# chlhnu/DOT-SOCP

Hardware: AMD Instinct MI355X
Metric: ADMM iters/sec on NxNxT dot2d staggered grid at 1/2/4/8 MI355X (higher is better)
Workload: dtype f64

## Files before the change

dot-socp_amd/capi.py:

```python
import ctypes
import os

import numpy as np

_HERE = os.path.dirname(os.path.abspath(__file__))
LIB_PATH = os.path.join(_HERE, "lib", "libdotsocp.so")

i64 = ctypes.c_longlong
dbl = ctypes.c_double
vp = ctypes.c_void_p


class DotsocpError(RuntimeError):
    def __init__(self, code, msg):
        super().__init__(f"libdotsocp error {code}: {msg}")
        self.code = code


class Problem(ctypes.Structure):
    _fields_ = [("dim", ctypes.c_int), ("weighted", ctypes.c_int),
                ("ny", i64), ("nx", i64), ("nt", i64),
                ("D", dbl), ("E", dbl), ("cScale", dbl), ("dScale", dbl),
                ("normc", dbl), ("normd", dbl)]


class Opts(ctypes.Structure):
    _fields_ = [("tau", dbl), ("sigma", dbl), ("tol", dbl), ("maxit", i64),
                ("ifCheckStepByStep", ctypes.c_int), ("checkPrimDualFeas", ctypes.c_int),
                ("scaling", ctypes.c_int), ("time_limit", dbl)]


class Result(ctypes.Structure):
    _fields_ = [("sigma", dbl), ("sigma_internal", dbl), ("cScale", dbl), ("dScale", dbl),
                ("times", dbl * 7), ("iters", i64), ("hist_len", i64), ("stopped", ctypes.c_int),
                ("time_extra", dbl)]


class AccOpts(ctypes.Structure):
    _fields_ = [("restart", i64), ("rho", dbl), ("theta", dbl)]


METHOD_INPALM, METHOD_PALM, METHOD_ACCADMM = 0, 1, 2


F_PHI, F_Q, F_ALPHA, F_Z, F_BETA, F_C, F_WEIGHT = range(7)

SYMBOLS = {
    "dotsocp_last_error": (ctypes.c_char_p, []),
    "dotsocp_version": (ctypes.c_char_p, []),
    "dotsocp_device_count": (ctypes.c_int, []),
    "dotsocp_proj_soc": (ctypes.c_int, [vp, vp, i64, i64]),
    "dotsocp_bfd": (ctypes.c_int, [vp, vp, i64, i64, i64, dbl, dbl]),
    "dotsocp_bfd_conj": (ctypes.c_int, [vp, vp, i64, i64, i64, dbl]),
    "dotsocp_bfd1d": (ctypes.c_int, [vp, vp, i64, i64, dbl, dbl]),
    "dotsocp_bfd_conj1d": (ctypes.c_int, [vp, vp, i64, i64, dbl]),
    "dotsocp_oper_poisson": (ctypes.c_int, [vp, vp, i64, i64, i64, dbl]),
    "dotsocp_dctn": (ctypes.c_int, [vp, i64, i64, i64, ctypes.c_int]),
    "dotsocp_proj_soc_dev": (ctypes.c_int, [vp, vp, i64, i64, vp]),
    "dotsocp_bfd_dev": (ctypes.c_int, [vp, vp, i64, i64, i64, dbl, dbl, vp]),
    "dotsocp_bfd_conj_dev": (ctypes.c_int, [vp, vp, i64, i64, i64, dbl, vp]),
    "dotsocp_create": (vp, [ctypes.POINTER(Problem), ctypes.c_int, ctypes.c_int]),
    "dotsocp_create_multi": (vp, [ctypes.POINTER(Problem), ctypes.c_int, ctypes.c_int]),
    "dotsocp_destroy": (None, [vp]),
    "dotsocp_rccl_unique_id": (ctypes.c_int, [vp]),
    "dotsocp_attach_rccl": (ctypes.c_int, [vp, vp, ctypes.c_int, ctypes.c_int]),
    "dotsocp_slab_range": (ctypes.c_int, [i64, ctypes.c_int, ctypes.c_int, ctypes.POINTER(i64), ctypes.POINTER(i64)]),
    "dotsocp_field_len": (i64, [ctypes.POINTER(Problem), ctypes.c_int]),
    "dotsocp_dct_algorithm": (ctypes.c_int, [i64]),
    "dotsocp_release_cache": (i64, []),
    "dotsocp_upload": (ctypes.c_int, [vp, ctypes.c_int, vp]),
    "dotsocp_upload_layers": (ctypes.c_int, [vp, ctypes.c_int, vp, i64, i64]),
    "dotsocp_download": (ctypes.c_int, [vp, ctypes.c_int, vp]),
    "dotsocp_begin": (ctypes.c_int, [vp, ctypes.POINTER(Opts)]),
    "dotsocp_begin_method": (ctypes.c_int, [vp, ctypes.POINTER(Opts), ctypes.c_int, ctypes.POINTER(AccOpts)]),
    "dotsocp_run": (ctypes.c_int, [vp, i64, ctypes.POINTER(i64)]),
    "dotsocp_recover_outputs": (ctypes.c_int, [vp, vp, vp, vp, vp, vp, vp, vp, vp]),
    "dotsocp_jump_next_level": (ctypes.c_int, [vp, vp]),
    "dotsocp_finish": (ctypes.c_int, [vp, ctypes.POINTER(Result)]),
    "dotsocp_get_history": (ctypes.c_int, [vp, vp, vp, vp, vp]),
    "dotsocp_set_profiling": (ctypes.c_int, [vp, ctypes.c_int]),
    "dotsocp_kernel_time": (ctypes.c_int, [vp, ctypes.c_char_p, ctypes.POINTER(dbl), ctypes.POINTER(i64)]),
    "dotsocp_canary_check": (ctypes.c_int, []),
    "dotsocp_synchronize": (ctypes.c_int, [vp]),
}

_lib = None


def _share_torchs_hip_runtime():
    import importlib.util
    import sys
    if "torch" in sys.modules or os.environ.get("DOTSOCP_SYSTEM_HIP"):
        return
    try:
        spec = importlib.util.find_spec("torch")
    except (ImportError, ValueError):
        return
    if not spec or not spec.submodule_search_locations:
        return
    for name in ("libamdhip64.so", "libamdhip64.so.7"):
        path = os.path.join(list(spec.submodule_search_locations)[0], "lib", name)
        if os.path.exists(path):
            try:
                ctypes.CDLL(path, mode=ctypes.RTLD_GLOBAL)
            except OSError:
                pass
            return


def lib():
    global _lib
    if _lib is None:
        _share_torchs_hip_runtime()
        if not os.path.exists(LIB_PATH):
            raise ImportError(
                f"{LIB_PATH} is missing: build the HIP extension first "
                "(python -c 'import __graft_entry__ as g; g.build()'); there is no CPU fallback")
        L = ctypes.CDLL(LIB_PATH)
        for name, (res, args) in SYMBOLS.items():
            f = getattr(L, name)
            f.restype = res
            f.argtypes = args
        _lib = L
    return _lib


def check(code):
    if code != 0:
        raise DotsocpError(code, lib().dotsocp_last_error().decode())


def fptr(a):
    if not isinstance(a, np.ndarray) or a.dtype != np.float64 or not (a.flags.f_contiguous or a.flags.c_contiguous):
        raise ValueError("expected a contiguous float64 numpy array")
    return a.ctypes.data


def slab_range(nt, world, rank):
    t0, t1 = i64(), i64()
    check(lib().dotsocp_slab_range(nt, world, rank, ctypes.byref(t0), ctypes.byref(t1)))
    return t0.value, t1.value


def rccl_unique_id():
    buf = (ctypes.c_ubyte * 128)()
    check(lib().dotsocp_rccl_unique_id(buf))
    return bytes(buf)


DCT_ALGORITHMS = ("none", "fft", "pfa", "rader", "bluestein", "dense")

# ... 4 lines not shown
```

dot-socp_amd/csrc/capi.hip:

```cpp
#include <cstring>
#include <new>

#include "comm.h"
#include "solver.h"

using namespace dotsocp;

namespace dotsocp {
extern thread_local std::string g_last_error;
int dotsocp_slab_range_impl(i64 nt, int world, int rank, i64 *t0, i64 *t1);
}

struct dotsocp_ctx {
    Solver s;
};

static int require_device() {
    int n = 0;
    if (hipGetDeviceCount(&n) != hipSuccess || n <= 0) {
        set_error("no HIP device available (libdotsocp has no CPU fallback)");
        return DOTSOCP_ENODEVICE;
    }
    return 0;
}
// ... 171 lines not shown
    DS_ARG(res && rhs && ny >= 1 && nx >= 1 && nt >= 1, "bad array");
    DS_CHECK(require_device());
    const i64 n = ny * nx * nt;
    DevBuf da, db, cy, cx, ct;
    Plans pl;
    DS_CHECK(da.alloc(n));
    DS_CHECK(db.alloc(n));
    DS_CHECK(pl.make(ny, nx, nt));
    const double pi = 3.14159265358979323846;
    auto table = [&](DevBuf &d, i64 m) -> int {
        std::vector<double> t((size_t)m);
        for (i64 k = 0; k < m; ++k) t[k] = (2.0 * (double)(m - 1) * (double)(m - 1)) * (1.0 - cos(pi * (double)k / (double)m));
        DS_CHECK(d.alloc(m));
        DS_HIP(hipMemcpy(d.p, t.data(), sizeof(double) * m, hipMemcpyHostToDevice));
        return 0;
    };
    DS_CHECK(table(cy, ny));
    DS_CHECK(table(cx, nx));
    DS_CHECK(table(ct, nt));
    DS_HIP(hipMemcpy(da.p, rhs, sizeof(double) * n, hipMemcpyHostToDevice));
    Grid g;
    g.set(ny, nx, nt, 0, nt);
    DS_CHECK(launch_dct_axis(pl.py, da.p, db.p, ny, nx, nt, 0, 0, nullptr));
    DS_CHECK(launch_dct_axis(pl.px, db.p, da.p, ny, nx, nt, 1, 0, nullptr));
    DS_CHECK(launch_poisson_t_single(pl.pt, g, kernelScale, cy.p, cx.p, ct.p, da.p, db.p, 0, nullptr, tsolve_tri_allowed()));
    DS_CHECK(launch_dct_axis(pl.px, da.p, db.p, ny, nx, nt, 1, 1, nullptr));
    DS_CHECK(launch_dct_axis(pl.py, db.p, da.p, ny, nx, nt, 0, 1, nullptr));
    DS_HIP(hipDeviceSynchronize());
    DS_HIP(hipMemcpy(res, da.p, sizeof(double) * n, hipMemcpyDeviceToHost));
    return 0;
}

dotsocp_ctx *dotsocp_create(const dotsocp_problem *prob, int device, int nslabs) {
    dotsocp_ctx *c = new (std::nothrow) dotsocp_ctx();
    if (!c) { set_error("out of host memory"); return nullptr; }
    if (c->s.init(prob, device, nslabs) != 0) {
        delete c;
        return nullptr;
    }
    return c;
}

dotsocp_ctx *dotsocp_create_multi(const dotsocp_problem *prob, int first_device, int ngpu) {
    dotsocp_ctx *c = new (std::nothrow) dotsocp_ctx();
    if (!c) { set_error("out of host memory"); return nullptr; }
    if (c->s.init(prob, first_device, ngpu, true) != 0) {
        delete c;
        return nullptr;
    }
    return c;
}

void dotsocp_destroy(dotsocp_ctx *ctx) { delete ctx; }

int dotsocp_slab_range(dotsocp_i64 nt, int world, int rank, dotsocp_i64 *t0, dotsocp_i64 *t1) {
    DS_ARG(t0 && t1 && world >= 1 && rank >= 0 && rank < world && nt >= 2 * world, "bad slab request");
    return dotsocp_slab_range_impl(nt, world, rank, t0, t1);
}

int dotsocp_rccl_unique_id(unsigned char id[128]) {
    DS_ARG(id != nullptr, "id is NULL");
    Rccl &api = rccl_api();
    DS_CHECK(api.load());
    ncclUniqueId uid;
    static_assert(sizeof(uid) == 128, "ncclUniqueId is expected to be 128 bytes");
    DS_NCCL(api.GetUniqueId(&uid));
    memcpy(id, &uid, sizeof uid);
    return 0;
}

int dotsocp_attach_rccl(dotsocp_ctx *ctx, const unsigned char id[128], int rank, int world) {
    if (!ctx) { set_error("ctx is NULL"); return DOTSOCP_EINVAL; }
    return ctx->s.attach_rccl(id, rank, world);
}

#define CTX_OR_FAIL()                                      \
    do {                                                   \
        if (!ctx) { set_error("ctx is NULL"); return DOTSOCP_EINVAL; } \
        (void)hipGetLastError();    \
    } while (0)

int dotsocp_dct_algorithm(dotsocp_i64 n) { return dct_choose_algorithm(n); }

dotsocp_i64 dotsocp_field_len(const dotsocp_problem *p, int field) {
    if (!p || (p->dim != 1 && p->dim != 2) || p->nt < 2 || p->nx < 1 || (p->dim == 2 && p->ny < 1)) return -1;
    const i64 ny = p->dim == 1 ? p->nx : p->ny, nx = p->dim == 1 ? 1 : p->nx, nt = p->nt;
    const i64 Nphi = ny * nx * nt, Nz = ny * nx * (nt - 1);
    const i64 Nq = Nz + ny * (nx - 1) * nt + (ny - 1) * nx * nt;
    switch (field) {
        case DOTSOCP_F_PHI: case DOTSOCP_F_C: return Nphi;
        case DOTSOCP_F_Q: case DOTSOCP_F_ALPHA: case DOTSOCP_F_WEIGHT: return Nq;
        case DOTSOCP_F_Z: case DOTSOCP_F_BETA: return Nz * (p->dim == 1 ? 6 : 10);
        default: return -1;
    }
}

int dotsocp_upload(dotsocp_ctx *ctx, int field, const double *host) { CTX_OR_FAIL(); return ctx->s.upload(field, host); }
dotsocp_i64 dotsocp_release_cache(void) { return (dotsocp_i64)device_cache_release(); }

int dotsocp_upload_layers(dotsocp_ctx *ctx, int field, const double *host, dotsocp_i64 t0, dotsocp_i64 n) {
    CTX_OR_FAIL();
    return ctx->s.upload_layers(field, host, t0, n);
}
int dotsocp_download(dotsocp_ctx *ctx, int field, double *host) { CTX_OR_FAIL(); return ctx->s.download(field, host); }
int dotsocp_begin(dotsocp_ctx *ctx, const dotsocp_opts *opts) { CTX_OR_FAIL(); return ctx->s.begin(opts); }
int dotsocp_begin_method(dotsocp_ctx *ctx, const dotsocp_opts *opts, int method, const dotsocp_acc_opts *acc) {
    CTX_OR_FAIL();
    return ctx->s.begin_method(opts, method, acc);
}
int dotsocp_recover_outputs(dotsocp_ctx *ctx, const double *rho0, const double *rho1, double *rho, double *Ex,
                            double *Ey, double *q0, double *bx, double *by) {
    CTX_OR_FAIL();
    if (ctx->s.prob.dim == 1)
        return ctx->s.recover_outputs(rho0, rho1, rho, nullptr, Ex, q0, nullptr, bx);
    return ctx->s.recover_outputs(rho0, rho1, rho, Ex, Ey, q0, bx, by);
}

int dotsocp_jump_next_level(dotsocp_ctx *coarse, dotsocp_ctx *fine) {
    if (!coarse || !fine) { set_error("context is NULL"); return DOTSOCP_EINVAL; }
    return fine->s.jump_from(coarse->s);
}

int dotsocp_run(dotsocp_ctx *ctx, dotsocp_i64 n_iters, dotsocp_i64 *done) { CTX_OR_FAIL(); return ctx->s.run(n_iters, done); }
int dotsocp_finish(dotsocp_ctx *ctx, dotsocp_result *res) { CTX_OR_FAIL(); return ctx->s.finish(res); }

int dotsocp_get_history(dotsocp_ctx *ctx, double *kkt, double *time, double *iter, double *pdGap) {
    CTX_OR_FAIL();
    const Solver &s = ctx->s;
    const size_t n = s.hist_iter.size();
    for (size_t i = 0; i < n; ++i) {
        if (kkt) for (int j = 0; j < 7; ++j) kkt[j * n + i] = s.hist_kkt[i * 7 + j];
        if (time) time[i] = s.hist_time[i];
        if (iter) iter[i] = s.hist_iter[i];
        if (pdGap) pdGap[i] = s.hist_gap[i];
    }
    return 0;
}

int dotsocp_set_profiling(dotsocp_ctx *ctx, int on) {
    CTX_OR_FAIL();
    ctx->s.profiling = on != 0;
    return 0;
}

int dotsocp_kernel_time(dotsocp_ctx *ctx, const char *name, double *avg_ms, dotsocp_i64 *launches) {
    CTX_OR_FAIL();
    DS_ARG(name != nullptr, "name is NULL");
    static const char *names[PH_COUNT] = {"rhs", "poisson", "cone_proj", "qstep", "beta", "kkt",
                                          "cone_fused_a", "cone_fused_b", "materialise", "comm",
                                          "interp", "acc_cone", "acc_gather", "qstep_first", "transpose"};
    for (int i = 0; i < PH_COUNT; ++i)
        if (strcmp(name, names[i]) == 0) {
            const i64 n = ctx->s.phase_launches[i];
            if (avg_ms) *avg_ms = n ? ctx->s.phase_ms[i] / (double)n : 0.0;
            if (launches) *launches = n;
            return 0;
        }
    set_error("unknown kernel family '%s'", name);
    return DOTSOCP_EINVAL;
}

int dotsocp_canary_check(void) {
    std::string rep;
    const int bad = canary_check(&rep);
    if (bad) set_error("canary: %d device buffer(s) written out of bounds: %s", bad, rep.c_str());
    return bad;
}

int dotsocp_synchronize(dotsocp_ctx *ctx) {
    CTX_OR_FAIL();
    ctx->s.cur_dev = -1;
    return ctx->s.sync_all();
}

}
```

dot-socp_amd/csrc/cone.hip:

```cpp
#include "device_utils.h"
#include "kernels.h"

namespace dotsocp {


template <int K>
__global__ void __launch_bounds__(256) k_proj_soc(double *__restrict__ out, const double *__restrict__ in, i64 M) {
    for (i64 i = (i64)blockIdx.x * blockDim.x + threadIdx.x; i < M; i += (i64)gridDim.x * blockDim.x) {
        double v[K];
#pragma unroll
        for (int j = 0; j < K; ++j) v[j] = in[j * M + i];
        proj_row<K>(v);
#pragma unroll
        for (int j = 0; j < K; ++j) out[j * M + i] = v[j];
    }
}

__global__ void __launch_bounds__(256) k_proj_soc_any(double *__restrict__ out, const double *__restrict__ in, i64 M,
                                                      i64 K) {
    for (i64 i = (i64)blockIdx.x * blockDim.x + threadIdx.x; i < M; i += (i64)gridDim.x * blockDim.x) {
        double x1 = in[i];
        const double n = sqrt(soc_norm2([&](i64 j) { return in[j * M + i]; }, K));
        double c = (x1 / n + 1.0) * 0.5;
        c = (c > 1.0) ? 1.0 : c;
// ... 30 lines not shown
    const double q0 = q[i];
    z[i] = dF - s * q0;
    z[9 * g.Nc + i] = dF + s * q0;
    const double *bx = q + g.offBx;
    const double *by = q + g.offBy;
#pragma unroll
    for (int dt = 0; dt < 2; ++dt) {
        const i64 tt = tl + dt;
        if (x >= 1) z[(1 + 2 * dt) * g.Nc + i] = sf * bx[g.bxLayer * tt + y + g.py * (x - 1)];
        if (x <= g.nx - 2) z[(2 + 2 * dt) * g.Nc + i] = sf * bx[g.bxLayer * tt + y + g.py * x];
        if (y >= 1) z[(5 + 2 * dt) * g.Nc + i] = sf * by[g.byLayer * tt + (y - 1) + g.pyb * x];
        if (y <= g.ny - 2) z[(6 + 2 * dt) * g.Nc + i] = sf * by[g.byLayer * tt + y + g.pyb * x];
    }
}

int launch_bfd(const Grid &g, double *z, const double *q, double s, double dF, hipStream_t st) {
    if (g.Nz <= 0) return 0;
    DS_KLAUNCH(k_bfd, cell_grid(g, g.ncl), dim3(TILE_Y, TILE_X), 0, st, g, z, q, s, edge_factor(s), dF);
    DS_HIP(hipGetLastError());
    return 0;
}

__global__ void __launch_bounds__(TILE_Y *TILE_X) k_bfd_conj(Grid g, double *__restrict__ q, const double *__restrict__ w,
                                                              double s, double sf, int seg,
                                                              const double *__restrict__ tail_bx,
                                                              const double *__restrict__ tail_by) {
    const i64 y = (i64)blockIdx.x * TILE_Y + threadIdx.x;
    const i64 x = (i64)blockIdx.y * TILE_X + threadIdx.y;
    const i64 tl = blockIdx.z;
    WPlain W{w, g.Nc};
    if (seg == 0) {
        if (y >= g.ny || x >= g.nx) return;
        const i64 i = y + g.py * (x + g.nx * tl);
        q[i] = s * (w[9 * g.Nc + i] - w[i]);
    } else if (seg == 1) {
        if (y >= g.ny || x >= g.nx - 1) return;
        q[g.offBx + g.bxLayer * tl + y + g.py * x] = sf * gather_bx(g, W, y, x, tl, tail_bx);
    } else {
        if (y >= g.ny - 1 || x >= g.nx) return;
        q[g.offBy + g.byLayer * tl + y + g.pyb * x] = sf * gather_by(g, W, y, x, tl, tail_by);
    }
}

int launch_bfd_conj(const Grid &g, double *q, const double *w, double s, hipStream_t st, const double *tail_bx,
                    const double *tail_by) {
    const double sf = edge_factor(s);
    if (!g.first && (!tail_bx || !tail_by)) {
        set_error("bfd_conj on a time slab needs the left neighbour's tails");
        return DOTSOCP_EINVAL;
    }
    const dim3 blk(TILE_Y, TILE_X);
    if (g.Nz > 0) DS_KLAUNCH(k_bfd_conj, cell_grid(g, g.ncl), blk, 0, st, g, q, w, s, sf, 0, tail_bx, tail_by);
    if (g.bxLayer > 0) DS_KLAUNCH(k_bfd_conj, cell_grid(g, g.ntl), blk, 0, st, g, q, w, s, sf, 1, tail_bx, tail_by);
    if (g.byLayer > 0) DS_KLAUNCH(k_bfd_conj, cell_grid(g, g.ntl), blk, 0, st, g, q, w, s, sf, 2, tail_bx, tail_by);
    DS_HIP(hipGetLastError());
    return 0;
}

#define MARCH 8

template <int MODE>
__global__ void __launch_bounds__(TILE_Y *TILE_X) k_cone_march(Grid g, LoopCoef c, const double *__restrict__ q,
                                                                const double *zin, const double *betain,
                                                                double *zout, double *betaout) {
    const i64 y = (i64)blockIdx.x * TILE_Y + threadIdx.x;
    const i64 x = (i64)blockIdx.y * TILE_X + threadIdx.y;
    if (y >= g.ny || x >= g.nx) return;
    const i64 tbeg = (i64)blockIdx.z * MARCH;
    const i64 tend = (tbeg + MARCH < g.ncl) ? tbeg + MARCH : g.ncl;
    EdgeQuad cur = load_edges(g, q, y, x, tbeg, c.sf);
    for (i64 tl = tbeg; tl < tend; ++tl) {
        const i64 i = y + g.py * (x + g.nx * tl);
        const EdgeQuad nxt = load_edges(g, q, y, x, tl + 1, c.sf);
        double v[10];
        build_z2(v, q[i], cur, nxt, c.s, c.dF);
        if (MODE == 0) {
#pragma unroll
            for (int j = 0; j < 10; ++j) v[j] = v[j] - betain[j * g.Nc + i];
            proj_row<10>(v);
#pragma unroll
            for (int j = 0; j < 10; ++j) zout[j * g.Nc + i] = v[j];
        } else {
#pragma unroll
            for (int j = 0; j < 10; ++j) {
                const double r = zin[j * g.Nc + i] - v[j];
                betaout[j * g.Nc + i] = betain[j * g.Nc + i] + c.tau * r;
            }
        }
        cur = nxt;
    }
}

static inline dim3 march_grid(const Grid &g) {
    return dim3((unsigned)((g.ny + TILE_Y - 1) / TILE_Y), (unsigned)((g.nx + TILE_X - 1) / TILE_X),
                (unsigned)((g.ncl + MARCH - 1) / MARCH));
}

int launch_cone_proj(const Grid &g, const LoopCoef &c, const double *q, const double *beta, double *z,
                     hipStream_t st) {
    if (g.Nz <= 0) return 0;
    DS_KLAUNCH(k_cone_march<0>, march_grid(g), dim3(TILE_Y, TILE_X), 0, st, g, c, q, (const double *)nullptr,
                       beta, z, (double *)nullptr);
    DS_HIP(hipGetLastError());
    return 0;
}

int launch_beta_update(const Grid &g, const LoopCoef &c, const double *q, const double *z, double *beta,
                       hipStream_t st) {
    if (g.Nz <= 0) return 0;
    DS_KLAUNCH(k_cone_march<1>, march_grid(g), dim3(TILE_Y, TILE_X), 0, st, g, c, q, z, (const double *)beta,
                       (double *)nullptr, beta);
    DS_HIP(hipGetLastError());
    return 0;
}

__global__ void __launch_bounds__(TILE_Y *TILE_X) k_gather_tail(Grid g, const double *__restrict__ z,
                                                                 const double *__restrict__ beta,
                                                                 double *__restrict__ tail_bx,
                                                                 double *__restrict__ tail_by) {
    const i64 y = (i64)blockIdx.x * TILE_Y + threadIdx.x;
    const i64 x = (i64)blockIdx.y * TILE_X + threadIdx.y;
    const i64 tl = g.ncl - 1;
    auto w = [&](int j, i64 cell) { return z[j * g.Nc + cell] + beta[j * g.Nc + cell]; };
    if (y < g.ny && x < g.nx - 1) {
        double acc = w(3, y + g.py * ((x + 1) + g.nx * tl));
        acc += w(4, y + g.py * (x + g.nx * tl));
        tail_bx[y + g.py * x] = acc;
    }
    if (y < g.ny - 1 && x < g.nx) {
        double acc = w(7, (y + 1) + g.py * (x + g.nx * tl));
        acc += w(8, y + g.py * (x + g.nx * tl));
        tail_by[y + g.pyb * x] = acc;
    }
}

int launch_gather_tail(const Grid &g, const double *z, const double *beta, double *tail_bx, double *tail_by,
                       hipStream_t st) {
    if (g.ncl <= 0) return 0;
    DS_KLAUNCH(k_gather_tail, cell_grid(g, 1), dim3(TILE_Y, TILE_X), 0, st, g, z, beta, tail_bx, tail_by);
    DS_HIP(hipGetLastError());
    return 0;
}

}
```

dot-socp_amd/csrc/device_utils.h:

```cpp
#pragma once
#include "common.h"

namespace dotsocp {

#define TILE_Y 64
#define TILE_X 4

__device__ __forceinline__ i64 xcd_tile(unsigned b, unsigned nb) {
    const unsigned full = nb >> 3, rem = nb & 7u, r = b & 7u, q = b >> 3;
    return (i64)r * full + (r < rem ? r : rem) + q;
}

struct BlockId {
    unsigned x, y, z;
};
__device__ __forceinline__ BlockId block_id(bool remap) {
    BlockId b{blockIdx.x, blockIdx.y, blockIdx.z};
    if (remap) {
        const unsigned nb = gridDim.x * gridDim.y * gridDim.z;
        const i64 L = xcd_tile(b.x + gridDim.x * (b.y + gridDim.y * b.z), nb);
        b.x = (unsigned)(L % gridDim.x);
        b.y = (unsigned)((L / gridDim.x) % gridDim.y);
        b.z = (unsigned)(L / ((i64)gridDim.x * gridDim.y));
    }
    return b;
}

__device__ __forceinline__ void lds_barrier() { asm volatile("s_waitcnt lgkmcnt(0)\n\ts_barrier" ::: "memory"); }

__device__ __forceinline__ void glds16(const void *gsrc, unsigned lds_dst) {
    unsigned keep;
    asm volatile("s_mov_b32 %0, m0\n\ts_mov_b32 m0, %2\n\ts_nop 0\n\tglobal_load_lds_dwordx4 %1, off\n\ts_mov_b32 m0, %0"
                 : "=&s"(keep)
                 : "v"(gsrc), "s"(lds_dst)
                 : "memory");
}

template <bool NT>
__device__ __forceinline__ double ld_stream(const double *p) { return NT ? __builtin_nontemporal_load(p) : *p; }
template <bool NT>
__device__ __forceinline__ void st_stream(double *p, double v) {
    if (NT) __builtin_nontemporal_store(v, p);
    else *p = v;
}
bool stream_nt_enabled();

template <class X, class I>
__device__ __forceinline__ double soc_norm2(const X &x, I K) {
    const I lim = (K - 2) & ~(I)3;
    double p = x(1) * x(1);
    I j = 2;
#pragma unroll
    for (; j - 1 < lim; j += 4) {
        const double a = x(j), b = x(j + 1), c = x(j + 2), d = x(j + 3);
        p += (a * a + b * b) + (c * c + d * d);
    }
#pragma unroll
    for (; j < K; ++j) p += x(j) * x(j);
    return p;
}

template <int K>
__device__ __forceinline__ void proj_row(double (&v)[K]) {
    const double n = sqrt(soc_norm2([&](int j) { return v[j]; }, K));
    double c = (v[0] / n + 1.0) * 0.5;
    c = (c > 1.0) ? 1.0 : c;
    c = (c < 0.0) ? 0.0 : c;
#pragma unroll
    for (int j = 1; j < K; ++j) v[j] = c * v[j];
    v[0] = (c >= 1.0) ? v[0] : c * n;
}

struct EdgeQuad {
    double xm, xp, ym, yp;
};

__device__ __forceinline__ EdgeQuad load_edges(const Grid &g, const double *__restrict__ q, i64 y, i64 x,
                                               i64 tt, double sf) {
    const double *bx = (g.nx >= 2) ? q + g.offBx + g.bxLayer * tt : q;
    const double *by = (g.ny >= 2) ? q + g.offBy + g.byLayer * tt : q;
    const i64 nxe = (g.nx >= 2) ? g.nx - 2 : 0, nye = (g.ny >= 2) ? g.ny - 2 : 0;
    const i64 rowy = (g.ny >= 2) ? g.pyb : 0;
    const i64 xm = (x >= 1) ? x - 1 : 0, xp = (x <= nxe) ? x : nxe;
    const i64 ym = (y >= 1) ? y - 1 : 0, yp = (y <= nye) ? y : nye;
    const double vxm = bx[y + g.py * xm], vxp = bx[y + g.py * xp];
    const double vym = by[ym + rowy * x], vyp = by[yp + rowy * x];
    EdgeQuad e;
    e.xm = (x >= 1) ? sf * vxm : 0.0;
    e.xp = (x <= g.nx - 2) ? sf * vxp : 0.0;
    e.ym = (y >= 1) ? sf * vym : 0.0;
    e.yp = (y <= g.ny - 2) ? sf * vyp : 0.0;
    return e;
}

__device__ __forceinline__ void build_z2(double (&v)[10], double q0, const EdgeQuad &a, const EdgeQuad &b,
                                         double s, double dF) {
    v[0] = dF - s * q0;
    v[1] = a.xm; v[2] = a.xp; v[3] = b.xm; v[4] = b.xp;
    v[5] = a.ym; v[6] = a.yp; v[7] = b.ym; v[8] = b.yp;
    v[9] = dF + s * q0;
}

template <class W>
__device__ __forceinline__ double gather_bx(const Grid &g, const W &w, i64 y, i64 xe, i64 tl,
                                            const double *__restrict__ tail_bx) {
    double acc = 0.0;
    if (tl < g.ncl) {
        acc += w(1, y + g.py * ((xe + 1) + g.nx * tl));
        acc += w(2, y + g.py * (xe + g.nx * tl));
    }
    if (tl >= 1) {
        acc += w(3, y + g.py * ((xe + 1) + g.nx * (tl - 1)));
        acc += w(4, y + g.py * (xe + g.nx * (tl - 1)));
    } else if (!g.first) {
        acc += tail_bx[y + g.py * xe];
    }
    return acc;
}

template <class W>
__device__ __forceinline__ double gather_by(const Grid &g, const W &w, i64 ye, i64 x, i64 tl,
                                            const double *__restrict__ tail_by) {
    double acc = 0.0;
    if (tl < g.ncl) {
        acc += w(5, (ye + 1) + g.py * (x + g.nx * tl));
        acc += w(6, ye + g.py * (x + g.nx * tl));
    }
    if (tl >= 1) {
        acc += w(7, (ye + 1) + g.py * (x + g.nx * (tl - 1)));
        acc += w(8, ye + g.py * (x + g.nx * (tl - 1)));
    } else if (!g.first) {
        acc += tail_by[ye + g.pyb * x];
    }
    return acc;
}

struct WPlain {
    const double *w;
    i64 Nz;
    __device__ __forceinline__ double operator()(int j, i64 cell) const { return w[j * Nz + cell]; }
};

struct RhsArgs {
    Grid g;
    double at, ax, ay;
    const double *q, *alpha, *cvec, *weight, *u0_prev;
};

template <bool WEIGHTED>
__device__ __forceinline__ double rhs_value(const RhsArgs &a, i64 y, i64 x, i64 tl) {
    const Grid &g = a.g;
    auto u = [&](i64 k) { return WEIGHTED ? a.weight[k] * a.q[k] - a.alpha[k] : a.q[k] - a.alpha[k]; };
    const i64 node = y + g.py * (x + g.nx * tl);
    double r = 0.0;
    if (tl >= 1)
        r += a.at * u(node - g.plane);
    else if (!g.first)
        r += a.at * a.u0_prev[y + g.py * x];
    if (tl < g.ncl) r += (-a.at) * u(node);
    const i64 bxo = g.offBx + g.bxLayer * tl;
    if (x >= 1) r += a.ax * u(bxo + y + g.py * (x - 1));
    if (x <= g.nx - 2) r += (-a.ax) * u(bxo + y + g.py * x);
    const i64 byo = g.offBy + g.byLayer * tl;
    if (y >= 1) r += a.ay * u(byo + (y - 1) + g.pyb * x);
    if (y <= g.ny - 2) r += (-a.ay) * u(byo + y + g.pyb * x);
    return r + a.cvec[node];
}

}
```

dot-socp_amd/csrc/fused.hip:

```cpp
#include "device_utils.h"
#include "gather_tile.h"
#include "kernels.h"

#include <cstdlib>

namespace dotsocp {

template <int MODE, int XB, bool NT = false>
__global__ void __launch_bounds__(64 * XB) k_cone_fused(Grid g, LoopCoef c, FusedArgs a) {
    constexpr bool DUAL = (MODE >= 5);
    constexpr bool UPD = (MODE != 0 && MODE != 6);
    constexpr bool PROJ = (MODE < 2 || MODE >= 5);
    __shared__ double2 xch[2][XB][64];
    __shared__ double2 xchp[DUAL ? 2 : 1][DUAL ? XB : 1][DUAL ? 64 : 1];
    const int lane = threadIdx.x, xl = threadIdx.y;
    const BlockId blk = block_id(a.xcd != 0);
    const i64 y = (i64)blk.x * 64 + lane;
    const i64 x = (i64)blk.y * XB + xl;
    const bool inb = (y < g.ny) && (x < g.nx);
    const i64 yc = inb ? y : 0, xc = inb ? x : 0;
    const i64 t0 = ((i64)blk.z + a.z0) * a.TC;
    const i64 t1 = (t0 + a.TC < g.ncl) ? t0 + a.TC : g.ncl;
    const bool lastChunk = (t1 == g.ncl);
    constexpr bool GATHER = (PROJ || MODE == 4);
    const bool carried = GATHER && !DUAL && t0 > 0 && a.carry_in != nullptr;
    const i64 tstart = (GATHER && t0 > 0 && !carried) ? t0 - 1 : t0;
    const i64 nxblk = gridDim.y, nyblk = gridDim.x;

    EdgeQuad cur = load_edges(g, a.q, yc, xc, tstart, c.sf), curo, cur3;
    if (UPD) curo = load_edges(g, a.q_old, yc, xc, tstart, c.sf);
    if (MODE == 5) cur3 = load_edges(g, a.q3, yc, xc, tstart, c.sf);
    GatherCarry gc, gcp;
    if (carried) {
        const i64 ci = yc + g.py * xc;
        gc.p3 = a.carry_in[ci]; gc.p4 = a.carry_in[g.plane + ci];
        gc.p7 = a.carry_in[2 * g.plane + ci]; gc.p8 = a.carry_in[3 * g.plane + ci];
    }
    const i64 tstop = (GATHER && lastChunk) ? t1 + 1 : t1;
    for (i64 tl = tstart; tl < tstop; ++tl) {
        const bool hasCell = tl < g.ncl;
        const bool own = tl >= t0;
        double w[10], wp[10];
        if (hasCell) {
            const i64 i = yc + g.py * (xc + g.nx * tl);
            const EdgeQuad nxt = load_edges(g, a.q, yc, xc, tl + 1, c.sf);
            double b[10], v[10];
#pragma unroll
            for (int j = 0; j < 10; ++j) b[j] = ld_stream<NT>(a.beta_in + j * g.Nc + i);
            if (a.bpend) {
#pragma unroll
                for (int j = 0; j < 10; ++j) b[j] = b[j] * a.bmul / a.bdiv;
                if (a.bpend > 1) {
#pragma unroll
                    for (int j = 0; j < 10; ++j) b[j] = b[j] * a.bmul2 / a.bdiv2;
                }
            }
            build_z2(v, a.q[i], cur, nxt, c.s, c.dF);
            if (UPD) {
                const EdgeQuad nxto = load_edges(g, a.q_old, yc, xc, tl + 1, c.sf);
                double zo[10];
                build_z2(zo, a.q_old[i], curo, nxto, c.s, c.dF);
#pragma unroll
                for (int j = 0; j < 10; ++j) zo[j] = zo[j] - b[j];
                proj_row<10>(zo);
#pragma unroll
                for (int j = 0; j < 10; ++j) {
                    const double r = zo[j] - v[j];
                    b[j] = b[j] + c.tau * r;
                }
                if (own && inb) {
                    if (MODE != 3) {
#pragma unroll
                        for (int j = 0; j < 10; ++j) st_stream<NT>(a.beta_out + j * g.Nc + i, b[j]);
                    }
                    if (MODE == 2 || MODE == 3) {
#pragma unroll
                        for (int j = 0; j < 10; ++j) st_stream<NT>(a.z_out + j * g.Nc + i, zo[j]);
                    }
                }
                curo = nxto;
                if (MODE == 4) {
#pragma unroll
                    for (int j = 0; j < 10; ++j) w[j] = zo[j] + b[j];
                    if (own && inb) a.q2[i] = c.s * (w[9] - w[0]);
                }
            }
            cur = nxt;
            if (PROJ) {
                if (MODE == 5) {
                    const EdgeQuad nxt3 = load_edges(g, a.q3, yc, xc, tl + 1, c.sf);
                    build_z2(v, a.q3[i], cur3, nxt3, c.s, c.dF);
                    cur3 = nxt3;
                }
#pragma unroll
                for (int j = 0; j < 10; ++j) v[j] = v[j] - b[j];
                proj_row<10>(v);
#pragma unroll
                for (int j = 0; j < 10; ++j) w[j] = v[j] + b[j];
                if (own && inb) a.q2[i] = c.s * (w[9] - w[0]);
                if (DUAL) {
#pragma unroll
                    for (int j = 0; j < 10; ++j) wp[j] = w[j] + c.tau * v[j];
                    if (own && inb) a.p2[i] = c.s * (wp[9] - wp[0]);
                }
            }
        } else {
#pragma unroll
            for (int j = 0; j < 10; ++j) w[j] = 0.0;
            if (DUAL) {
#pragma unroll
                for (int j = 0; j < 10; ++j) wp[j] = 0.0;
            }
        }
        if constexpr (GATHER && !DUAL)
            gather_emit<XB>(g, c.sf, xch, gc, w, tl, own && inb, x, y, xl, lane, nxblk, nyblk, blk.y, blk.x,
                            a.q2, a.sx, a.sy);
        if constexpr (DUAL) {
            gather_post<XB>(xch, gc, w, xl, lane);
            gather_post<XB>(xchp, gcp, wp, xl, lane);
            __syncthreads();
            gather_finish<XB>(g, c.sf, xch, gc, w, tl, own && inb, x, y, xl, lane, nxblk, nyblk, blk.y, blk.x,
                              a.q2, a.sx, a.sy);
            gather_finish<XB>(g, c.sf, xchp, gcp, wp, tl, own && inb, x, y, xl, lane, nxblk, nyblk, blk.y, blk.x,
                              a.p2, a.sxp, a.syp);
        }
    }
    if (GATHER && !DUAL && !lastChunk && a.carry_out != nullptr && inb) {
        const i64 ci = y + g.py * x;
        a.carry_out[ci] = gc.p3; a.carry_out[g.plane + ci] = gc.p4;
        a.carry_out[2 * g.plane + ci] = gc.p7; a.carry_out[3 * g.plane + ci] = gc.p8;
    }
}

bool stream_nt_enabled() {
    const char *e = getenv("DOTSOCP_NT");
    return !(e && atoi(e) == 0);
}

bool tile_xcd_remap(const Grid &g) {
    return (g.py % 16) != 0;
}

bool cone_split_enabled() { return true; }

int fused_geometry(const Grid &g, FusedGeom &fg) {
    fg.XB = 4;
    fg.nyblk = (g.ny + 63) / 64;
    fg.nxblk = (g.nx + fg.XB - 1) / fg.XB;
    const i64 tiles = fg.nyblk * fg.nxblk;
    const i64 target = 2048;
    i64 chunks = (target + tiles - 1) / tiles;
    if (chunks < 1) chunks = 1;
    if (!(g.first && g.last) && cone_split_enabled() && chunks < 2 && g.ncl >= 12) chunks = 2;
    i64 TC = (g.ncl + chunks - 1) / chunks;
    if (TC < 8) TC = 8;
    if (TC > g.ncl) TC = g.ncl;
    if (TC < 1) TC = 1;
    fg.TC = TC;
    fg.chunks = (g.ncl + TC - 1) / TC;
    fg.sx_len = (g.ncl + 1) * fg.nxblk * g.ny;
    fg.sy_len = (g.ncl + 1) * g.nx * fg.nyblk;
    return 0;
}

int launch_cone_fused(int mode, const Grid &g, const LoopCoef &c, const FusedGeom &fg, FusedArgs a,
                      hipStream_t st, i64 z0, i64 zcount) {
    if (g.Nz <= 0) return 0;
    if (zcount < 0) zcount = fg.chunks - z0;
    if (z0 < 0 || zcount <= 0 || z0 + zcount > fg.chunks) return 0;
    a.TC = fg.TC;
    a.z0 = (int)z0;
    a.xcd = tile_xcd_remap(g) ? 1 : 0;
    dim3 grid((unsigned)fg.nyblk, (unsigned)fg.nxblk, (unsigned)zcount);
    dim3 blk(64, 4);
    const bool nt = stream_nt_enabled();
#define CONE_MODE(M)                                                                     \
    case M:                                                                              \
        if (nt) DS_KLAUNCH((k_cone_fused<M, 4, true>), grid, blk, 0, st, g, c, a);       \
        else DS_KLAUNCH((k_cone_fused<M, 4>), grid, blk, 0, st, g, c, a);                \
        break;
    switch (mode) {
        CONE_MODE(0) CONE_MODE(1) CONE_MODE(2) CONE_MODE(3) CONE_MODE(4) CONE_MODE(5) CONE_MODE(6)
#undef CONE_MODE
        default: set_error("bad fused mode"); return DOTSOCP_EINVAL;
    }
    DS_HIP(hipGetLastError());
    return 0;
}

}
```

dot-socp_amd/csrc/kernels.h:

```cpp
#pragma once
#include "common.h"
#include "defer.h"

namespace dotsocp {

struct LoopCoef {
    double s;
    double sf;
    double dF;
    double at, ax, ay;
    double tau;
    double c1, c2;
    double dinv1, dinv2;
};

enum {
    S_Q2 = 0, S_Z2, S_APHI2, S_ALPHA2, S_BETA2, S_FBBETA2, S_PRIM1, S_PRIM2, S_DUAL1, S_DUAL2,
    S_COMPLEM, S_DOTCOMP, S_RHO2, S_RHOFQ2, S_MRHOB, S_M2, S_RHOB2, S_QALPHA, S_CPHI, S_PHI2,
    S_COUNT
};

struct KktCoef {
    double sigma;
    double kappa;
    double dsD;
    double dsE;
};

int launch_proj_soc(double *out, const double *in, i64 M, i64 K, hipStream_t st);
int launch_bfd(const Grid &g, double *z, const double *q, double s, double dF, hipStream_t st);
int launch_bfd_conj(const Grid &g, double *q, const double *w, double s, hipStream_t st, const double *tail_bx = nullptr,
                    const double *tail_by = nullptr);
int launch_cone_proj(const Grid &g, const LoopCoef &c, const double *q, const double *beta, double *z,
                     hipStream_t st);
int launch_beta_update(const Grid &g, const LoopCoef &c, const double *q, const double *z, double *beta,
                       hipStream_t st);
int launch_gather_tail(const Grid &g, const double *z, const double *beta, double *tail_bx, double *tail_by,
                       hipStream_t st);

struct FusedGeom {
    int XB;
    i64 nyblk, nxblk;
    i64 TC, chunks;
    i64 sx_len, sy_len;
};
struct FusedArgs {
    const double *q_old;
    const double *q;
    const double *beta_in;
    double *beta_out;
    double *z_out;
    double *q2;
    double *sx, *sy;
    const double *q3;
    double *p2, *sxp, *syp;
    i64 TC;
    int bpend;
    double bmul, bdiv;
    double bmul2, bdiv2;
    int xcd;
    int z0;
    const double *carry_in;
    double *carry_out;
};
bool tile_xcd_remap(const Grid &g);
int fused_geometry(const Grid &g, FusedGeom &fg);
int launch_cone_fused(int mode, const Grid &g, const LoopCoef &c, const FusedGeom &fg, FusedArgs a,
                      hipStream_t st, i64 z0 = 0, i64 zcount = -1);
bool cone_split_enabled();

struct KktWork;
struct AccArgs {
    const double *q;
    const double *z_in, *beta_in;
    const double *z0, *beta0;
    double *z0_out, *beta0_out;
    double bdiv;
    KktCoef kk;
    const double *alpha_p, *weight;
    double *partials;
    int nostore;
    double *z_out, *beta_out;
    double *q2, *sx, *sy;
    i64 TC;
    double c1, c2, om_rho, rho;
};
struct AccCoef {
    double c1, c2, om_rho, rho;
    double om_c1, c1c2;
};
int launch_acc_cone(int mode, const Grid &g, const LoopCoef &c, const FusedGeom &fg, AccArgs a, hipStream_t st);
int launch_acc_cone_kkt(const Grid &g, const LoopCoef &c, const FusedGeom &fg, AccArgs a, const KktWork &w, hipStream_t st);
int launch_acc_restart(double *x, const double *xp, double *anchor, i64 n, const AccCoef &k, double div, hipStream_t st);
int launch_acc_interp(double *x, const double *xp, double *aux, i64 n, const AccCoef &k, int mode, int write_aux,
                      hipStream_t st);

int launch_prolong_phi(const Grid &gf, const Grid &gc, const double *phic, double *phif, double sc_in, double sc_out,
                       hipStream_t st, i64 tc0 = 0);
int launch_prolong_beta(const Grid &gf, const Grid &gc, const double *betac, double *betaf, double *neg, double sc_in0,
                        double sc_in1, double sc_out, hipStream_t st, i64 tc0 = 0, i64 Nzc = -1);
int launch_scale_div(double *x, const double *w, i64 n, double sc, hipStream_t st);
int launch_fill(double *x, i64 n, double v, hipStream_t st);
int launch_outputs(const Grid &g, const double *q, const double *alpha, const double *weight, const double *rho0,
                   const double *rho1, const double *a_prev, double sig, double cD, double dD, int which, double *out,
                   hipStream_t st);
int launch_out_tail(const Grid &g, const double *alpha, const double *weight, double sig, double cD, double *out,
                    hipStream_t st);

int launch_qstep_fused(const Grid &g, const LoopCoef &c, const FusedGeom &fg, const double *phi,
                       const double *q2, const double *sx, const double *sy, const double *weight,
                       const double *tail_bx, const double *tail_by, double *q_out, double *alpha,
                       hipStream_t st);
struct QStepExtra {
    int apend;
    double amul, adiv;
    double *partials, *resid;
    double kappa, dsD;
    double *u0_tail;
};
int launch_qstep_rhs(const Grid &g, const LoopCoef &c, const FusedGeom &fg, const double *phi, const double *q2,
                     const double *sx, const double *sy, const double *weight, const double *tail_bx,
                     const double *tail_by, const double *cvec, double *q_out, const double *alpha_in, double *alpha_out,
                     double *rhs, hipStream_t st, i64 z0 = 0, i64 zcount = -1, i64 zstride = 1,
                     const QStepExtra *ex = nullptr);
i64 qstep_rhs_blocks(const Grid &g, const FusedGeom &fg);
int launch_rhs_sigma_fix(double *rhs, const double *r, double *cvec, i64 n, double factor, hipStream_t st);
i64 qstep_rhs_chunks(const Grid &g, const FusedGeom &fg, i64 *TC = nullptr);
int launch_qstep_rhs_acc(int var, const Grid &g, const LoopCoef &c, const FusedGeom &fg, const double *phi,
                         const double *q2, const double *sx, const double *sy, const double *weight, const double *cvec,
                         double *q_raw, const double *alpha_in, double *alpha_out, double *rhs, double *q_state,
                         const double *q_anchor, const double *alpha_anchor, const AccCoef &k, hipStream_t st,
                         const double *tail_bx = nullptr, const double *tail_by = nullptr, double *u0_tail = nullptr);
int launch_rhs_fixup(const Grid &g, const LoopCoef &c, const double *u0_prev, double *rhs, hipStream_t st);
int launch_qstep_palm_first(const Grid &g, const LoopCoef &c, const FusedGeom &fg, const double *phi, const double *q2,
                            const double *sx, const double *sy, const double *cvec, double *q_out, const double *alpha,
                            double *rhs, hipStream_t st, const double *tail_bx = nullptr, const double *tail_by = nullptr,
                            const double *qk = nullptr);
int launch_grad(const Grid &g, const LoopCoef &c, const double *phi, double *out, hipStream_t st);
int launch_tail_finalize(const Grid &g, const LoopCoef &c, const FusedGeom &fg, const double *q2, const double *sx,
                         const double *sy, double *tail_bx, double *tail_by, hipStream_t st);
int launch_kkt_tail(const Grid &g, const double *alpha, const double *beta, const double *weight, double *a0,
                    double *a0w, double *bt_bx, double *bt_by, hipStream_t st);
int launch_rhs(const Grid &g, const LoopCoef &c, const double *q, const double *alpha, const double *cvec,
               const double *weight, const double *u0_prev, double *rhs, hipStream_t st);
int launch_qstep(const Grid &g, const LoopCoef &c, const double *phi, const double *z, const double *beta,
                 const double *weight, const double *tail_bx, const double *tail_by, double *q,
                 double *alpha, hipStream_t st);
int launch_u0_tail(const Grid &g, const double *q, const double *alpha, const double *weight, double *out,
                   hipStream_t st);
int launch_scale(double *x, i64 n, double mul, double div, hipStream_t st);
#define DS_MAX_WORLD 64
struct PencilCuts {
    int world;
    i64 cut[DS_MAX_WORLD + 1];
};
int launch_pencil_pack(bool pack, const PencilCuts &pc, i64 plane, i64 ntl, double *slab, double *stage, hipStream_t st);

#define TRI_EXTRA 256
int launch_tri_local(const Grid &g, i64 nt, double kscale, const double *cy, const double *cx, const PencilCuts &pc,
                     const double *r, double *send, hipStream_t st);
int launch_tri_reduced(const Grid &g, i64 nt, double kscale, const double *cy, const double *cx, const PencilCuts &pc,
                       int rank, i64 l0, i64 nl, const i64 *slab_n, const double *recv, double *back, double *zero_work,
                       hipStream_t st, const double *own_recv = nullptr, double *own_back = nullptr);
int launch_tri_final(const Grid &g, i64 nt, double kscale, const double *cy, const double *cx, const PencilCuts &pc,
                     const double *back, double *x, hipStream_t st);
bool tsolve_tri_supported(i64 nt);
bool tsolve_tri_preferred(i64 nt, bool pow2, i64 plane);
int launch_tsolve_tri(const Grid &g, i64 nt, double kscale, const double *cy, const double *cx, double *x, hipStream_t st);
struct GatherMsgs {
    const double *src[DS_MAX_WORLD];
    double *dst[DS_MAX_WORLD];
    i64 count[DS_MAX_WORLD];
    int n;
};
int launch_gather_msgs(const GatherMsgs &m, hipStream_t st);

#define KKT_SLICES 64
struct KktWork {
    double *partials;
    i64 maxBlocks;
    double *sums;
};
struct KktHalo {
    const double *a0_prev, *a0w_prev, *btail_bx, *btail_by;
};
i64 kkt_partials_needed(const Grid &g);
int launch_kkt(const Grid &g, const LoopCoef &c, const KktCoef &k, const double *phi, const double *q,
               const double *alpha, const double *z, const double *beta, const double *cvec,
               const double *weight, const KktHalo &halo, const KktWork &w, int parts, hipStream_t st,
               bool layer0 = false, double *resid = nullptr);
int launch_kkt_nodual(const Grid &g, const LoopCoef &c, const KktCoef &k, const double *phi, const double *q,
                      const double *alpha, const double *cvec, const double *weight, const KktWork &w, hipStream_t st);
int launch_kkt_bnd_dual(const Grid &g, const LoopCoef &c, const KktCoef &k, const FusedGeom &fg, const double *q,
                        const double *alpha, const double *weight, const double *q2, const double *sx, const double *sy,
                        const KktWork &w, hipStream_t st);
int launch_kkt_cells_update(const Grid &g, const LoopCoef &c, const KktCoef &k, const FusedGeom &fg, FusedArgs a,
                            const double *phi, const double *alpha, const double *weight, const KktWork &w,
                            hipStream_t st, bool edges = false, const double *q_new = nullptr);
int launch_norms(const Grid &g, const LoopCoef &c, const KktCoef &k, const FusedGeom &fg, FusedArgs a, const double *phi,
                 const double *alpha, const double *weight, const KktWork &w, hipStream_t st);
double *kkt_qstep_partials(const Grid &g, const KktWork &w);
int launch_kkt_final(const Grid &g, const KktWork &w, hipStream_t st);

enum { DCT_ALG_NONE = 0, DCT_ALG_FFT = 1, DCT_ALG_PFA = 2, DCT_ALG_RADER = 3, DCT_ALG_BLUESTEIN = 4, DCT_ALG_DENSE = 5 };
int dct_choose_algorithm(i64 n);
struct DctPlan;
DctPlan *dct_plan_create(i64 n);
void dct_plan_destroy(DctPlan *p);
int launch_dct_axis(const DctPlan *p, const double *src, double *dst, i64 n0, i64 n1, i64 n2, int axis,
                    int inverse, hipStream_t st, i64 pitch0 = 0);
bool dct_plan_is_pow2(const DctPlan *p);
bool dct_plan_has_tsolve(const DctPlan *p);
int launch_dct_t_solve(const DctPlan *p, const double *src, double *dst, i64 ny, i64 nplane, i64 line0, i64 nl,
                       i64 nt, double kscale, const double *cy, const double *cx, const double *ct, hipStream_t st,
                       i64 pitch0 = 0);
int launch_spectral_divide_pencil(double *data, i64 ny, i64 line0, i64 nl, i64 nt, double kscale, const double *cy,
                                  const double *cx, const double *ct, hipStream_t st);
int launch_spectral_divide(double *data, i64 ny, i64 nt, i64 x0, i64 nxl, double kscale, const double *cy,
                           const double *cx, const double *ct, hipStream_t st, i64 pitch0 = 0);
bool tsolve_tri_allowed();
int launch_poisson_t_single(const DctPlan *pt, const Grid &g, double kscale, const double *cy, const double *cx,
                            const double *ct, double *p, double *p2, i64 pitch0, hipStream_t st, bool allow_tri);

}
```

dot-socp_amd/csrc/kkt.hip:

```cpp
#include "device_utils.h"
#include "gather_tile.h"
#include "kernels.h"

#include <cstdlib>

namespace dotsocp {

struct WBeta {
    const double *b;
    i64 Nz;
    __device__ __forceinline__ double operator()(int j, i64 cell) const { return b[j * Nz + cell]; }
};

template <bool WEIGHTED, int PART, bool NODUAL = false>
__global__ void __launch_bounds__(TILE_Y *TILE_X) k_kkt(Grid g, LoopCoef c, KktCoef k, i64 chunk,
                                                         const double *__restrict__ phi, const double *__restrict__ q,
                                                         const double *__restrict__ alpha, const double *__restrict__ z,
                                                         const double *__restrict__ beta,
                                                         const double *__restrict__ cvec,
                                                         const double *__restrict__ weight,
                                                         KktHalo halo, double *__restrict__ partials,
                                                         double *__restrict__ resid) {
    const i64 y = (i64)blockIdx.x * TILE_Y + threadIdx.x;
    const i64 x = (i64)blockIdx.y * TILE_X + threadIdx.y;
// ... 128 lines not shown
                const double m = k.kappa * (wgt(idx) * alpha[idx]);
                const double d = m - rb;
                S[S_MRHOB] += d * d;
                S[S_M2] += m * m;
                S[S_RHOB2] += rb * rb;
            }
        }
    }
    __shared__ double red[TILE_X][S_COUNT];
    const int lane = threadIdx.x;
#pragma unroll
    for (int i = 0; i < S_COUNT; ++i) {
        double v = S[i];
#pragma unroll
        for (int off = 32; off >= 1; off >>= 1) v += __shfl_down(v, off, 64);
        if (lane == 0) red[threadIdx.y][i] = v;
    }
    __syncthreads();
    if (threadIdx.y == 0 && lane < S_COUNT) {
        double v = red[0][lane];
#pragma unroll
        for (int wv = 1; wv < TILE_X; ++wv) v += red[wv][lane];
        const i64 b = blockIdx.x + (i64)gridDim.x * (blockIdx.y + (i64)gridDim.y * blockIdx.z);
        partials[b * S_COUNT + lane] = v;
    }
}

template <bool WEIGHTED, bool EDGES, bool NORMS = false, bool NT = false>
__global__ void __launch_bounds__(TILE_Y *TILE_X) k_kkt_cells(Grid g, LoopCoef c, KktCoef k, FusedArgs a,
                                                               const double *__restrict__ phi,
                                                               const double *__restrict__ alpha,
                                                               const double *__restrict__ weight,
                                                               double *__restrict__ partials) {
    __shared__ double2 xch[EDGES ? 2 : 1][EDGES ? TILE_X : 1][EDGES ? 64 : 1];
    const int lane = threadIdx.x, xl = threadIdx.y;
    const i64 y = (i64)blockIdx.x * TILE_Y + lane;
    const i64 x = (i64)blockIdx.y * TILE_X + xl;
    const bool inb = (y < g.ny) && (x < g.nx);
    const i64 yc = inb ? y : 0, xc = inb ? x : 0;
    const i64 t0 = (i64)blockIdx.z * a.TC;
    const i64 t1 = (t0 + a.TC < g.ncl) ? t0 + a.TC : g.ncl;
    const bool lastChunk = (t1 == g.ncl);
    const i64 tstart = (EDGES && t0 > 0) ? t0 - 1 : t0;
    const i64 tstop = (EDGES && lastChunk) ? t1 + 1 : t1;
    const i64 nxblk = gridDim.y, nyblk = gridDim.x;
    double S[S_COUNT];
#pragma unroll
    for (int i = 0; i < S_COUNT; ++i) S[i] = 0.0;
    auto wgt = [&](i64 idx) { return WEIGHTED ? weight[idx] : 1.0; };
    double p3 = 0.0, p4 = 0.0, p7 = 0.0, p8 = 0.0;
    int par = 0;
    if (inb || EDGES) {
        EdgeQuad cur = load_edges(g, a.q, yc, xc, tstart, c.sf);
        EdgeQuad curo = load_edges(g, a.q_old, yc, xc, tstart, c.sf);
        for (i64 tl = tstart; tl < tstop; ++tl) {
            const bool hasCell = tl < g.ncl;
            const bool own = (tl >= t0) && inb;
            double b[10];
            if (hasCell) {
                const i64 i = yc + g.py * (xc + g.nx * tl);
                const EdgeQuad nxt = load_edges(g, a.q, yc, xc, tl + 1, c.sf);
                const EdgeQuad nxto = load_edges(g, a.q_old, yc, xc, tl + 1, c.sf);
                const double q0 = a.q[i];
                double v[10], zo[10];
#pragma unroll
                for (int j = 0; j < 10; ++j) b[j] = ld_stream<NT>(a.beta_in + j * g.Nc + i);
                if (a.bpend) {
#pragma unroll
                    for (int j = 0; j < 10; ++j) b[j] = b[j] * a.bmul / a.bdiv;
                    if (a.bpend > 1) {
#pragma unroll
                        for (int j = 0; j < 10; ++j) b[j] = b[j] * a.bmul2 / a.bdiv2;
                    }
                }
                build_z2(v, q0, cur, nxt, c.s, c.dF);
                build_z2(zo, a.q_old[i], curo, nxto, c.s, c.dF);
#pragma unroll
                for (int j = 0; j < 10; ++j) zo[j] = zo[j] - b[j];
                proj_row<10>(zo);
                double zs = 0.0, bs = 0.0, rs = 0.0;
#pragma unroll
                for (int j = 0; j < 10; ++j) {
                    const double r = zo[j] - v[j];
                    b[j] = b[j] + c.tau * r;
                    zs += zo[j] * zo[j];
                    bs += b[j] * b[j];
                    rs += r * r;
                }
                cur = nxt;
                curo = nxto;
                if (own && NORMS) {
                    S[S_Z2] += zs;
                    S[S_BETA2] += bs;
                }
                if (own && !NORMS) {
#pragma unroll
                    for (int j = 0; j < 10; ++j) st_stream<NT>(a.beta_out + j * g.Nc + i, b[j]);
                    auto xj = [&](int j) { return zo[j] - k.sigma * b[j]; };
                    const double n = sqrt(soc_norm2(xj, 10)), x0 = xj(0);
                    double cf = (x0 / n + 1.0) * 0.5;
                    cf = (cf > 1.0) ? 1.0 : cf;
                    cf = (cf < 0.0) ? 0.0 : cf;
                    const double p0 = (cf >= 1.0) ? x0 : cf * n;
                    double cs = (zo[0] - p0) * (zo[0] - p0);
#pragma unroll
                    for (int j = 1; j < 10; ++j) {
                        const double d = zo[j] - cf * xj(j);
                        cs += d * d;
                    }
                    S[S_Z2] += zs;
                    S[S_BETA2] += bs;
                    S[S_PRIM2] += rs;
                    S[S_COMPLEM] += cs;
                    const double w = wgt(i);
                    const double av = alpha[i];
                    const double rhoT = k.kappa * (w * av);
                    double sq = 0.0;
#pragma unroll
                    for (int j = 1; j < 9; ++j) {
                        const double e = k.dsE * v[j];
                        sq += e * e;
                    }
                    double rhoFq = rhoT + k.dsD * q0 + sq / 4.0;
                    rhoFq = (rhoFq < 0.0) ? 0.0 : rhoFq;
                    const double dd = rhoT - rhoFq;
                    S[S_DOTCOMP] += dd * dd;
                    S[S_RHO2] += rhoT * rhoT;
                    S[S_RHOFQ2] += rhoFq * rhoFq;
                    const double q2b = c.s * (b[9] - b[0]);
                    const double wa = w * av;
                    S[S_FBBETA2] += q2b * q2b;
                    const double r2 = q2b + wa;
                    S[S_DUAL2] += r2 * r2;
                    if (!EDGES) {
                        double tmp = (-c.at) * phi[i];
                        tmp += c.at * phi[i + g.plane];
                        const double wq = w * q0;
                        S[S_Q2] += q0 * q0;
                        S[S_ALPHA2] += av * av;
                        S[S_APHI2] += tmp * tmp;
                        const double r1 = tmp - wq;
                        S[S_PRIM1] += r1 * r1;
                        S[S_QALPHA] += wq * av;
                    }
                }
            } else {
#pragma unroll
                for (int j = 0; j < 10; ++j) b[j] = 0.0;
            }
            if (EDGES) {
                auto dual = [&](i64 e, double acc) {
                    const double gb = c.sf * acc;
                    S[S_FBBETA2] += gb * gb;
                    const double r2 = gb + wgt(e) * alpha[e];
                    S[S_DUAL2] += r2 * r2;
                };
                xch[par][xl][lane] = make_double2(b[1], p3);
                __syncthreads();
                const bool sumLayer = (tl < g.ntl) && !(tl == 0 && !g.first);
                if (own) {
                    if (x < g.nx - 1) {
                        const i64 e = g.offBx + g.bxLayer * tl + y + g.py * x;
                        if (xl < TILE_X - 1) {
                            if (sumLayer) {
                            const double2 r = xch[par][xl + 1][lane];
                            double acc = r.x + b[2];
                            acc += r.y;
// ... 338 lines not shown
```

dot-socp_amd/csrc/solver.h:

```cpp
#pragma once
#include <chrono>
#include <functional>
#include <memory>
#include <string>
#include <vector>

#include "hostmem.h"
#include "kernels.h"

namespace dotsocp {

int guarded_malloc(void **p, size_t bytes);
void guarded_free(void *p);
long long device_cache_release();
int canary_check(std::string *report);
bool canary_enabled();
bool stream_stress_enabled();
void stream_stress(hipStream_t st);

template <class T>
inline int dmalloc(T **p, i64 n) {
    *p = nullptr;
    if (n <= 0) n = 1;
    return guarded_malloc((void **)p, sizeof(T) * (size_t)n);
}

inline int dzalloc(double **p, i64 n, hipStream_t st) {
    DS_CHECK(dmalloc(p, n));
    DS_HIP(hipMemsetAsync(*p, 0, sizeof(double) * (size_t)(n > 0 ? n : 1), st));
    return 0;
}

inline void dfree(void *p) {
    if (p) guarded_free(p);
}

struct DevRes {
    int dev = 0;
    DctPlan *py = nullptr, *px = nullptr, *pt = nullptr;
    double *cy = nullptr, *cx = nullptr, *ct = nullptr;
};

#define DS_XEV 8
struct Slab {
    int index = 0;
    int dev = 0;
    hipStream_t st = nullptr;
    hipStream_t st_z = nullptr;
    hipEvent_t ev_fork = nullptr, ev_join = nullptr, ev_halo = nullptr;
    hipEvent_t ev_cjoin = nullptr;
    hipEvent_t xev[DS_XEV] = {nullptr};
    hipEvent_t ev_tri = nullptr;
    hipEvent_t ev_msg = nullptr, ev_got = nullptr;
    int xev_next = 0;
    DevRes *res = nullptr;
    double *h_sums = nullptr;
    Grid g;
    double *phi = nullptr;
    double *q = nullptr;
    double *alpha = nullptr;
    double *z = nullptr;
    double *beta = nullptr;
    double *c = nullptr;
    double *weight = nullptr;
    double *w0 = nullptr, *w1 = nullptr;
    i64 l0 = 0, nl = 0;
    double *pencil = nullptr, *pencil2 = nullptr;
    double *stage = nullptr;
    double *u0_prev = nullptr, *tail_bx = nullptr, *tail_by = nullptr;
    double *a0_prev = nullptr, *a0w_prev = nullptr, *btail_bx = nullptr, *btail_by = nullptr;
    double *send_plane = nullptr, *send_plane2 = nullptr, *send_bx = nullptr, *send_by = nullptr;
    KktWork kw{};
    double *q_old = nullptr, *q2 = nullptr, *beta2 = nullptr, *sx = nullptr, *sy = nullptr;
    double *q3 = nullptr, *p2 = nullptr, *sxp = nullptr, *syp = nullptr;
    double *send_pbx = nullptr, *send_pby = nullptr, *ptail_bx = nullptr, *ptail_by = nullptr;
    double *alpha2 = nullptr;
    double *tri_send = nullptr, *tri_recv = nullptr, *tri_bsend = nullptr, *tri_brecv = nullptr, *tri_zero = nullptr;
    double *carry = nullptr;
    FusedGeom fg{};
    double *phi_p = nullptr, *alpha_p = nullptr, *z_p = nullptr;
    double *phi_a = nullptr, *q_a = nullptr, *alpha_a = nullptr, *z_a = nullptr, *beta_a = nullptr;
};

#define FOR_SLABS(s) for (auto &s : slabs) if (int rc_use__ = use(s)) return rc_use__; else

bool if_adjust_sigma(double iter, double last_iter);

enum Phase { PH_RHS = 0, PH_POISSON, PH_PROJ, PH_QSTEP, PH_BETA, PH_KKT, PH_FUSED_A, PH_FUSED_B, PH_MATERIALISE,
             PH_COMM, PH_INTERP, PH_ACC_CONE, PH_ACC_GATHER, PH_QSTEP0, PH_TRANSPOSE, PH_COUNT };

struct Solver {
    dotsocp_problem prob{};
    int device = 0;
    i64 ny = 0, nx = 0, nt = 0;
    hipStream_t stream = nullptr;
    hipStream_t stream_z = nullptr;
    hipEvent_t ev_fork = nullptr, ev_join = nullptr, ev_halo = nullptr;
    bool multi_device = false;
    int ndev_visible = 1;
    std::vector<DevRes *> devres;
    int cur_dev = -1;
    int use(const Slab &s);
    int use_dev(int d);
    DevRes *res_for(int dev);
    int xcopy(Slab &from, const double *src, Slab &to, double *dst, i64 count);
    int xcopy2d(Slab &from, const double *src, size_t spitch, Slab &to, double *dst, size_t dpitch, size_t width,
                size_t height);
    i64 column_pad() const;
    i64 row_pitch() const;
    int sync_all();
    int copy_rows(double *dev, double *host, i64 rowlen, i64 pitch, i64 nrows, bool up, hipStream_t st);
    bool comm_z = false;
    bool comm_async = false;
    int comm_depth = 0;
    hipStream_t cst(const Slab &s) const { return comm_z ? s.st_z : s.st; }
    int comm_enter();
    int comm_leave();
    int comm_fork();
    int comm_mark(hipEvent_t Slab::*ev);
    int comm_wait(hipEvent_t Slab::*ev);
    bool overlap = false;
    std::vector<Slab> slabs;
    std::unique_ptr<DeferCtx> defer;
    int world = 1;
    int rank = 0;
    void *nccl = nullptr;
    int open_groups = 0;
    double *h_sums = nullptr;
    double *d_red = nullptr;

    bool begun = false, finished = false, stopped = false;
    dotsocp_opts opts{};
    bool checkPrimDualFeas = true;
    double time_limit = 3600.0;
    double sigma = 1.0, sigmaScale = 1.0;
    double cScale = 1.0, dScale = 1.0, D = 1.0, E = 1.0;
    double norm_c = 0.0, norm_d = 0.0;
    double h = 1.0;
    int rescale = 0, use_feasOrg = 0;
    double maxFeas = 0.0, relGap = 0.0, tol_feasOrg = 0.0;
    double lastSigmaIt = 0.0;
    i64 it = 0;
    LoopCoef lc{};
    std::vector<double> hist_kkt, hist_time, hist_iter, hist_gap;
    std::chrono::steady_clock::time_point t_begin;
    double elapsed_prev = 0.0;
    double elapsed_agreed = 0.0;

    bool profiling = false;
    bool fused = true;
    bool deferred = false;
    bool z_valid = true;
    bool z_prev_ok = false;
    int ensure_z();
    int bpend = 0;
    double bmul = 1.0, bdiv = 1.0, bmul2 = 1.0, bdiv2 = 1.0;
    int push_beta_op(double mul, double div);
    int zp_pend = 0;
    double zp_mul = 1.0, zp_div = 1.0, zp_mul2 = 1.0, zp_div2 = 1.0;
    double last_S[S_COUNT] = {0};
    double last_S_sigma = 1.0;
    i64 last_S_it = -1;
    int flush_beta();
    bool apend = false;
    double amul = 1.0, adiv = 1.0;
    int flush_alpha();
    int sigma_scale_folded(double factor);
    bool norm_cache = true;
    bool kkt_fold = true;
    KktCoef kkt_coef() const;
    void set_pending(FusedArgs &a) const {
        a.bpend = bpend; a.bmul = bmul; a.bdiv = bdiv; a.bmul2 = bmul2; a.bdiv2 = bdiv2;
    }
    struct Pending { hipEvent_t a, b; int phase; };
    std::vector<Pending> pending;
    std::vector<hipEvent_t> event_pool;
    double phase_ms[PH_COUNT] = {0};
    i64 phase_launches[PH_COUNT] = {0};

    ~Solver();
    int init(const dotsocp_problem *p, int device, int nslabs, bool multi_dev = false);
    int attach_rccl(const unsigned char *id, int rank, int world);
    int upload(int field, const double *host);
    int upload_layers(int field, const double *host, i64 t0, i64 n);
    int download(int field, double *host);
    int begin(const dotsocp_opts *o);
    int begin_method(const dotsocp_opts *o, int method, const dotsocp_acc_opts *acc);
    int run(i64 n_iters, i64 *done);
    int finish(dotsocp_result *res);

    int alloc_slabs(int first, int count);
    int ensure_alloc();
    void free_slabs();
    bool multi() const { return world > 1; }
    bool remote() const { return nccl != nullptr; }
    int step(bool *brk);
    int rescale_block();
    struct PhiHooks { std::function<int()> fill, behind; };
    int phase_phi(const PhiHooks *hooks = nullptr);
    int phase_z(int part = 0);
    int phase_z_tails();
    int make_tails();
    int send_tails();
    int send_phi_head();
    int ship_tails();
    int phase_q(int part = 0, bool kkt = false);
    int phase_mult();
    int materialise();
    int kkt_sums(double *S, bool folded = false);
    int reduce_sums(double *S);
    int norms_light(double *S);
    int kkt_block(bool adjustSigmaYes, bool timed_out, bool *brk, bool folded = false);
    int scale_state(double a_mul, double a_div, double q_div, bool with_c);
    void update_coef();
    double elapsed() const;
    void prof_begin(int phase, bool on_z = false);
    void prof_end(int phase, bool on_z = false);
    int prof_flush();
    int poisson_all(const PhiHooks *hooks = nullptr);
    int transpose(bool forward);
    int exchange_q_halo(bool with_u0);
    int ensure_halo();
    int exchange_u0_tail();
    int make_u0_tail();
    int group_begin();
    int group_end();
    bool tri_tsolve = true;
    int tri_alloc();
    int tri_exchange(bool back);
    int poisson_t_tridiag(const PhiHooks *hooks);
    const bool qrhs = true;
    bool rhs_valid = false;
    bool halo_pending = false;
    bool u0_fresh = false;
    bool u0_made = false;
    typedef std::function<double *(Slab &)> Sel;
    int shift(int dir, const Sel &src, const Sel &dst, i64 count);
// ... 39 lines not shown
```

dot-socp_amd/csrc/solver.hip:

```cpp
#include "solver.h"

#include <algorithm>
#include <cmath>
#include <cstring>

#include "comm.h"

namespace dotsocp {

thread_local std::string g_last_error;

static int make_eig_table(double **dev, i64 n, i64 len = 0);

void set_error(const char *fmt, ...) {
    char buf[1024];
    va_list ap;
    va_start(ap, fmt);
    vsnprintf(buf, sizeof buf, fmt, ap);
    va_end(ap);
    g_last_error = buf;
}

int Solver::use_dev(int d) {
    if (cur_dev == d) return 0;
// ... 855 lines not shown
    FOR_SLABS(s) DS_CHECK(launch_tri_final(s.g, nt, kscale, s.res->cy, s.res->cx, pc, s.tri_brecv, s.w0, s.st));
    return 0;
}

static const int k1dCols[6] = {0, 5, 6, 7, 8, 9};

i64 Solver::field_len(int field) const {
    i64 ntn = nt, ntc = nt - 1;
    if (remote()) { ntn = slabs[0].g.ntl; ntc = slabs[0].g.ncl; }
    const i64 Nz = ny * nx * ntc, Nphi = ny * nx * ntn;
    const i64 Nq = Nz + ny * (nx - 1) * ntn + (ny - 1) * nx * ntn;
    switch (field) {
        case DOTSOCP_F_PHI: case DOTSOCP_F_C: return Nphi;
        case DOTSOCP_F_Q: case DOTSOCP_F_ALPHA: case DOTSOCP_F_WEIGHT: return Nq;
        case DOTSOCP_F_Z: case DOTSOCP_F_BETA: return Nz * (prob.dim == 1 ? 6 : 10);
        default: return -1;
    }
}

int Solver::copy_rows(double *dev, double *host, i64 rowlen, i64 pitch, i64 nrows, bool up, hipStream_t st) {
    if (rowlen <= 0 || nrows <= 0) return 0;
    if (pitch == rowlen) {
        if (up) DS_HIP(ds_memcpy_async(dev, host, sizeof(double) * rowlen * nrows, hipMemcpyHostToDevice, st));
        else DS_HIP(ds_memcpy_async(host, dev, sizeof(double) * rowlen * nrows, hipMemcpyDeviceToHost, st));
        return 0;
    }
    if (up) DS_HIP(ds_memcpy2d_async(dev, sizeof(double) * pitch, host, sizeof(double) * rowlen, sizeof(double) * rowlen,
                                    (size_t)nrows, hipMemcpyHostToDevice, st));
    else DS_HIP(ds_memcpy2d_async(host, sizeof(double) * rowlen, dev, sizeof(double) * pitch, sizeof(double) * rowlen,
                                 (size_t)nrows, hipMemcpyDeviceToHost, st));
    return 0;
}

static int copy_field(Solver &S, int field, double *host, bool up) {
    const i64 ny = S.ny, nx = S.nx;
    i64 ntn = S.nt, ntc = S.nt - 1;
    if (S.remote()) { ntn = S.slabs[0].g.ntl; ntc = S.slabs[0].g.ncl; }
    const i64 hplane = ny * nx, hbx = ny * (nx - 1), hby = (ny - 1) * nx;
    const i64 NzG = hplane * ntc;
    const i64 bxG = NzG, byG = NzG + hbx * ntn;
    for (auto &s : S.slabs) {
        DS_CHECK(S.use(s));
        hipStream_t cur = s.st;
        const Grid &g = s.g;
        const i64 t0 = S.remote() ? 0 : g.t0;
        auto nodes = [&](double *dev, double *h, i64 layers) { return S.copy_rows(dev, h, ny, g.py, nx * layers, up, cur); };
        switch (field) {
            case DOTSOCP_F_PHI: DS_CHECK(nodes(s.phi, host + hplane * t0, g.ntl)); break;
            case DOTSOCP_F_C: DS_CHECK(nodes(s.c, host + hplane * t0, g.ntl)); break;
            case DOTSOCP_F_Q: case DOTSOCP_F_ALPHA: case DOTSOCP_F_WEIGHT: {
                double *d = field == DOTSOCP_F_Q ? s.q : (field == DOTSOCP_F_ALPHA ? s.alpha : s.weight);
                DS_CHECK(nodes(d, host + hplane * t0, g.ncl));
                DS_CHECK(S.copy_rows(d + g.offBx, host + bxG + hbx * t0, ny, g.py, (nx - 1) * g.ntl, up, cur));
                DS_CHECK(S.copy_rows(d + g.offBy, host + byG + hby * t0, ny - 1, g.pyb, nx * g.ntl, up, cur));
                break;
            }
            case DOTSOCP_F_Z: case DOTSOCP_F_BETA: {
                double *d = field == DOTSOCP_F_Z ? s.z : s.beta;
                const int K = S.prob.dim == 1 ? 6 : 10;
                if (up && S.prob.dim == 1) DS_HIP(ds_memset_async(d, 0, sizeof(double) * 10 * g.Nc, cur));
                for (int j = 0; j < K; ++j) {
                    const int pj = S.prob.dim == 1 ? k1dCols[j] : j;
                    DS_CHECK(nodes(d + pj * g.Nc, host + j * NzG + hplane * t0, g.ncl));
                }
                break;
            }
        }
    }
    DS_CHECK(S.sync_all());
    return 0;
}

int Solver::upload(int field, const double *host) {
    DS_ARG(host != nullptr, "host pointer is NULL");
    DS_ARG(field_len(field) >= 0, "unknown field");
    DS_ARG(field != DOTSOCP_F_WEIGHT || prob.weighted, "weight uploaded to an unweighted problem");
    if (begun) { set_error("upload() after begin()"); return DOTSOCP_ESTATE; }
    cur_dev = -1;
    DS_CHECK(use_dev(device));
    DS_CHECK(ensure_alloc());
    return copy_field(*this, field, const_cast<double *>(host), true);
}

int Solver::upload_layers(int field, const double *host, i64 t0, i64 n) {
    DS_ARG(host != nullptr, "host pointer is NULL");
    DS_ARG(field == DOTSOCP_F_PHI || field == DOTSOCP_F_C, "layer uploads serve the node fields (phi, c)");
    const i64 ntn = remote() ? slabs[0].g.ntl : nt;
    DS_ARG(t0 >= 0 && n >= 0 && t0 + n <= ntn, "layer range outside the field");
    if (begun) { set_error("upload() after begin()"); return DOTSOCP_ESTATE; }
    cur_dev = -1;
    DS_CHECK(use_dev(device));
    DS_CHECK(ensure_alloc());
    const i64 hplane = ny * nx;
    for (auto &s : slabs) {
        DS_CHECK(use(s));
        const Grid &g = s.g;
        const i64 base = remote() ? 0 : g.t0;
        const i64 lo = std::max(t0, base), hi = std::min(t0 + n, base + g.ntl);
        if (lo >= hi) continue;
        double *dev = (field == DOTSOCP_F_PHI ? s.phi : s.c) + g.plane * (lo - base);
        DS_CHECK(copy_rows(dev, const_cast<double *>(host) + hplane * (lo - t0), ny, g.py, nx * (hi - lo), true, s.st));
    }
    DS_CHECK(sync_all());
    return 0;
}

int Solver::download(int field, double *host) {
    DS_ARG(host != nullptr, "host pointer is NULL");
    DS_ARG(field_len(field) >= 0, "unknown field");
    DS_ARG(field != DOTSOCP_F_WEIGHT || prob.weighted, "no weight in an unweighted problem");
    cur_dev = -1;
    DS_CHECK(use_dev(device));
    DS_CHECK(ensure_alloc());
    if (field == DOTSOCP_F_Z || field == DOTSOCP_F_BETA) {
        DS_CHECK(ensure_z());
        DS_CHECK(flush_beta());
    }
    if (field == DOTSOCP_F_ALPHA) DS_CHECK(flush_alpha());
    host_first_touch(host, sizeof(double) * (size_t)field_len(field));
    DS_CHECK(copy_field(*this, field, host, false));
    if (finished && (field == DOTSOCP_F_ALPHA || field == DOTSOCP_F_BETA)) host_scale(host, field_len(field), sigma);
    return 0;
}

void Solver::prof_begin(int phase, bool on_z) {
    if (!profiling) return;
    (void)use_dev(device);
    hipStream_t st = on_z ? stream_z : stream;
    Pending p;
    p.phase = phase;
    auto get = [&]() {
        hipEvent_t e;
        if (!event_pool.empty()) { e = event_pool.back(); event_pool.pop_back(); }
        else (void)hipEventCreate(&e);
        return e;
    };
    p.a = get();
    p.b = get();
    (void)ds_event_record(p.a, st);
    pending.push_back(p);
}

void Solver::prof_end(int phase, bool on_z) {
    if (!profiling) return;
    (void)use_dev(device);
    hipStream_t st = on_z ? stream_z : stream;
    for (auto it2 = pending.rbegin(); it2 != pending.rend(); ++it2)
        if (it2->phase == phase) { (void)ds_event_record(it2->b, st); break; }
}

int Solver::prof_flush() {
    if (!profiling || pending.empty()) return 0;
    DS_CHECK(use_dev(device));
    DS_HIP(ds_stream_synchronize(stream_z));
    DS_HIP(ds_stream_synchronize(stream));
    for (auto &p : pending) {
        float ms = 0.f;
        if (hipEventElapsedTime(&ms, p.a, p.b) == hipSuccess) {
            phase_ms[p.phase] += ms;
            phase_launches[p.phase] += 1;
        }
        event_pool.push_back(p.a);
        event_pool.push_back(p.b);
    }
    pending.clear();
    return 0;
}

double Solver::elapsed() const {
    return elapsed_prev + std::chrono::duration<double>(std::chrono::steady_clock::now() - t_begin).count();
}

void Solver::update_coef() {
    lc.s = E / D;
    lc.sf = edge_factor(lc.s);
    lc.dF = E / dScale;
    const double ht = 1.0 / (double)(nt - 1);
    lc.at = D * (1.0 / ht);
    lc.ax = (nx > 1) ? D * (1.0 / (1.0 / (double)(nx - 1))) : 0.0;
    lc.ay = (ny > 1) ? D * (1.0 / (1.0 / (double)(ny - 1))) : 0.0;
    lc.tau = opts.tau;
    const double tmp = (E / D) * (E / D);
    if (prob.weighted) { lc.c1 = 2.0 * tmp; lc.c2 = tmp; }
    else { lc.c1 = 1.0 + 2.0 * tmp; lc.c2 = 1.0 + tmp; }
    lc.dinv1 = 1.0 / lc.c1;
    lc.dinv2 = 1.0 / lc.c2;
}

int Solver::flush_beta() {
    if (!bpend) return 0;
    FOR_SLABS(s) {
        DS_CHECK(launch_scale(s.beta, 10 * s.g.Nc, bmul, bdiv, s.st));
        if (bpend > 1) DS_CHECK(launch_scale(s.beta, 10 * s.g.Nc, bmul2, bdiv2, s.st));
    }
    bpend = 0;
    return 0;
}

int Solver::push_beta_op(double mul, double div) {
    if (bpend >= 2) DS_CHECK(flush_beta());
    if (bpend == 0) { bmul = mul; bdiv = div; }
    else { bmul2 = mul; bdiv2 = div; }
    bpend += 1;
    return 0;
}

int Solver::flush_alpha() {
    if (!apend) return 0;
    FOR_SLABS(s) DS_CHECK(launch_scale(s.alpha, s.g.NqAlloc, amul, adiv, s.st));
    apend = false;
    return 0;
}

int Solver::sigma_scale_folded(double factor) {
    DS_CHECK(flush_alpha());
    DS_CHECK(ensure_halo());
    u0_made = false;
    DS_CHECK(push_beta_op(1.0, factor));
    if (multi()) {
        FOR_SLABS(s) DS_CHECK(launch_scale(s.alpha, s.g.NqAlloc, 1.0, factor, s.st));
    } else {
        apend = true; amul = 1.0; adiv = factor;
    }
    u0_fresh = false;
    FOR_SLABS(s) DS_CHECK(launch_rhs_sigma_fix(s.w0, s.w1, s.c, s.g.Nphi, factor, s.st));
    return 0;
}

int Solver::scale_state(double a_mul, double a_div, double q_div, bool with_c) {
    DS_CHECK(flush_alpha());
    if (begun) DS_CHECK(ensure_halo());
    u0_made = false;
    u0_fresh = false;
    rhs_valid = false;
    if (fused && begun) {
        DS_CHECK(push_beta_op(a_mul, a_div));
    }
    FOR_SLABS(s) {
        const Grid &g = s.g;
        if (with_c) DS_CHECK(launch_scale(s.c, g.Nphi, a_mul, a_div, s.st));
        if (!acc_light) DS_CHECK(launch_scale(s.alpha, g.NqAlloc, a_mul, a_div, s.st));
        if (!(fused && begun) && !acc_light) DS_CHECK(launch_scale(s.beta, 10 * g.Nc, a_mul, a_div, s.st));
        if (q_div != 1.0) {
            DS_CHECK(launch_scale(s.q, g.NqAlloc, 1.0, q_div, s.st));
            if (!(fused && begun) || z_valid) DS_CHECK(launch_scale(s.z, 10 * g.Nc, 1.0, q_div, s.st));
        }
    }
    if (q_div != 1.0 && fused && begun && !z_valid) z_prev_ok = false;
    return 0;
}

int Solver::begin_method(const dotsocp_opts *o, int m, const dotsocp_acc_opts *acc) {
    if (begun) { set_error("begin() called twice"); return DOTSOCP_ESTATE; }
    if (m == DOTSOCP_METHOD_INPALM) return begin(o);
    DS_ARG(m == DOTSOCP_METHOD_ACCADMM || m == DOTSOCP_METHOD_PALM, "unknown method");
    DS_ARG(prob.dim == 2, "the reference has PALM and acc-ADMM loops for 2-D problems only");
    DS_ARG(!(m == DOTSOCP_METHOD_PALM && prob.weighted), "the reference has no weighted PALM loop");
    method = m;
    int rc = begin(o);
    if (rc != 0) { method = DOTSOCP_METHOD_INPALM; return rc; }
    return (m == DOTSOCP_METHOD_PALM) ? palm_begin() : acc_begin(acc);
}

int Solver::begin(const dotsocp_opts *o) {
    DS_ARG(o != nullptr, "opts is NULL");
    DS_ARG(o->maxit >= 0, "opts.maxit < 0");
    DS_ARG(o->sigma > 0, "opts.sigma must be positive");
    if (begun) { set_error("begin() called twice"); return DOTSOCP_ESTATE; }
    cur_dev = -1;
    DS_CHECK(use_dev(device));
    DS_CHECK(ensure_alloc());
    if (method == DOTSOCP_METHOD_ACCADMM) {
        DS_CHECK(acc_alloc());
        fused = false;
    }
    opts = *o;
    checkPrimDualFeas = (o->checkPrimDualFeas < 0) ? !prob.weighted : (o->checkPrimDualFeas != 0);
    time_limit = (o->time_limit > 0) ? o->time_limit : 3600.0;
    sigma = o->sigma;
    lastSigmaIt = -INFINITY;
    cScale = prob.cScale; dScale = prob.dScale; D = prob.D; E = prob.E;
    use_feasOrg = 0;
    tol_feasOrg = 5 * o->tol;
    rescale = o->scaling ? 1 : 0;
    maxFeas = INFINITY; relGap = INFINITY;
    h = 1.0 / ((double)nx * (double)ny * (double)nt);
    norm_c = prob.normc; norm_d = prob.normd;
    update_coef();
    DS_CHECK(scale_state(1.0, sigma, 1.0, true));
    DS_CHECK(exchange_q_halo(false));
    sigmaScale = 1.0;
    it = 0;
    stopped = false;
    deferred = false;
    z_valid = true;
    z_prev_ok = false;
    rhs_valid = false;
    last_S_it = -1;
    hist_kkt.clear(); hist_time.clear(); hist_iter.clear(); hist_gap.clear();
    for (int i = 0; i < PH_COUNT; ++i) { phase_ms[i] = 0; phase_launches[i] = 0; }
    if (canary_enabled() && getenv("DOTSOCP_CANARY_SELFTEST")) {
        Slab &s0 = slabs[0];
        DS_CHECK(use(s0));
        const double v = 1.0;
        DS_HIP(ds_memcpy_async(s0.c + s0.g.Nphi, &v, sizeof v, hipMemcpyHostToDevice, s0.st));
        DS_HIP(ds_stream_synchronize(s0.st));
    }
    begun = true;
    elapsed_prev = 0.0;
    elapsed_agreed = 0.0;
    t_begin = std::chrono::steady_clock::now();
    return 0;
}

int Solver::poisson_all(const PhiHooks *hooks) {
    const i64 plane = slabs[0].g.plane;
    const bool tp2 = dct_plan_has_tsolve(devres[0]->pt);
    FOR_SLABS(s) {
        const Grid &g = s.g;
        DS_CHECK(launch_dct_axis(s.res->py, s.w0, s.w1, g.ny, g.nx, g.ntl, 0, 0, s.st, g.py));
        DS_CHECK(launch_dct_axis(s.res->px, s.w1, s.w0, g.ny, g.nx, g.ntl, 1, 0, s.st, g.py));
    }
    bool tri = multi() && tri_tsolve && world <= DS_MAX_WORLD;
    for (auto &s : slabs) tri = tri && s.g.ntl <= TRI_EXTRA;
    if (tri) {
        DS_CHECK(poisson_t_tridiag(hooks));
    } else {
    if (hooks && hooks->fill) {
        prof_end(PH_POISSON);
        DS_CHECK(hooks->fill());
        prof_begin(PH_POISSON);
    }
    if (hooks && hooks->behind) DS_CHECK(hooks->behind());
    if (multi()) {
        prof_begin(PH_TRANSPOSE);
        DS_CHECK(transpose(true));
        prof_end(PH_TRANSPOSE);
    }
    FOR_SLABS(s) {
        double *p = multi() ? s.pencil : s.w0;
        double *p2 = multi() ? s.pencil2 : s.w1;
        if (!multi()) {
            DS_CHECK(launch_poisson_t_single(s.res->pt, s.g, D * D, s.res->cy, s.res->cx, s.res->ct, p, p2, s.g.py, s.st, tri_tsolve));
        } else if (tp2) {
            DS_CHECK(launch_dct_t_solve(s.res->pt, p, p, s.g.py, plane, s.l0, s.nl, nt, D * D, s.res->cy, s.res->cx, s.res->ct, s.st));
        } else {
            DS_CHECK(launch_dct_axis(s.res->pt, p, p2, s.nl, 1, nt, 2, 0, s.st));
            DS_CHECK(launch_spectral_divide_pencil(p2, s.g.py, s.l0, s.nl, nt, D * D, s.res->cy, s.res->cx, s.res->ct, s.st));
            DS_CHECK(launch_dct_axis(s.res->pt, p2, p, s.nl, 1, nt, 2, 1, s.st));
        }
    }
    if (multi()) {
        prof_begin(PH_TRANSPOSE);
        DS_CHECK(transpose(false));
        prof_end(PH_TRANSPOSE);
    }
    }
    FOR_SLABS(s) {
        const Grid &g = s.g;
        DS_CHECK(launch_dct_axis(s.res->px, s.w0, s.w1, g.ny, g.nx, g.ntl, 1, 1, s.st, g.py));
        DS_CHECK(launch_dct_axis(s.res->py, s.w1, s.phi, g.ny, g.nx, g.ntl, 0, 1, s.st, g.py));
    }
    return 0;
}

int Solver::phase_phi(const PhiHooks *hooks) {
    DS_CHECK(ensure_halo());
    if (multi() && !u0_fresh) {
        DS_CHECK(make_u0_tail());
        prof_begin(PH_COMM, comm_z);
        DS_CHECK(exchange_u0_tail());
        prof_end(PH_COMM, comm_z);
    }
    prof_begin(PH_RHS);
    if (!rhs_valid) {
        DS_CHECK(flush_alpha());
        FOR_SLABS(s) DS_CHECK(launch_rhs(s.g, lc, s.q, s.alpha, s.c, s.weight, s.u0_prev, s.w0, s.st));
    } else if (multi()) {
        FOR_SLABS(s)
            if (!s.g.first) DS_CHECK(launch_rhs_fixup(s.g, lc, s.u0_prev, s.w0, s.st));
    }
    rhs_valid = false;
    prof_end(PH_RHS);
    prof_begin(PH_POISSON);
    DS_CHECK(poisson_all(hooks));
    prof_end(PH_POISSON);
    return 0;
}

int Solver::phase_z(int part) {
    if (part != 1) DS_CHECK(ensure_halo());
    if (!fused) {
        prof_begin(PH_PROJ);
        FOR_SLABS(s) DS_CHECK(launch_cone_proj(s.g, lc, s.q, s.beta, s.z, s.st));
        prof_end(PH_PROJ);
        return 0;
    }
    const int ph = deferred ? PH_FUSED_B : PH_FUSED_A;
    z_valid = false;
    z_prev_ok = false;
    prof_begin(ph);
    FOR_SLABS(s) {
        FusedArgs a{};
        a.q = s.q;
        a.q2 = s.q2;
        a.sx = s.sx;
        a.sy = s.sy;
        a.beta_in = s.beta;
        set_pending(a);
        const i64 C = s.fg.chunks;
        const i64 z0 = (part == 2) ? C - 1 : 0;
        const i64 zc = (part == 0) ? C : ((part == 1) ? C - 1 : 1);
        if (deferred) {
            a.q_old = s.q_old;
            a.beta_out = s.beta2;
        }
        const int mode = deferred ? 1 : 0;
        if (s.carry && C > 1) {
            for (i64 z = z0; z < z0 + zc; ++z) {
                a.carry_in = (z > 0) ? s.carry : nullptr;
                a.carry_out = (z + 1 < C) ? s.carry : nullptr;
                DS_CHECK(launch_cone_fused(mode, s.g, lc, s.fg, a, s.st, z, 1));
            }
        } else {
            DS_CHECK(launch_cone_fused(mode, s.g, lc, s.fg, a, s.st, z0, zc));
        }
        if (deferred && part != 1) std::swap(s.beta, s.beta2);
    }
    prof_end(ph);
    if (part == 1) return 0;
    if (deferred) bpend = 0;
    return 0;
}

int Solver::phase_z_tails() {
    return fused ? ship_tails() : 0;
}

int Solver::make_tails() {
    if (!multi()) return 0;
    FOR_SLABS(s)
        if (!s.g.last) DS_CHECK(launch_tail_finalize(s.g, lc, s.fg, s.q2, s.sx, s.sy, s.send_bx, s.send_by, s.st));
    return 0;
}

int Solver::send_tails() {
    if (!multi()) return 0;
    prof_begin(PH_COMM, comm_z);
    DS_CHECK(group_begin());
    DS_CHECK(shift(+1, [](Slab &s) { return s.send_bx; }, [](Slab &s) { return s.tail_bx; }, slabs[0].g.bxLayer));
    DS_CHECK(shift(+1, [](Slab &s) { return s.send_by; }, [](Slab &s) { return s.tail_by; }, slabs[0].g.byLayer));
    DS_CHECK(group_end());
    prof_end(PH_COMM, comm_z);
    return 0;
}

int Solver::send_phi_head() {
    if (!multi()) return 0;
    prof_begin(PH_COMM, comm_z);
    DS_CHECK(shift(-1, [](Slab &s) { return s.phi; }, [](Slab &s) { return s.phi + s.g.plane * s.g.ntl; }, slabs[0].g.plane));
    prof_end(PH_COMM, comm_z);
    return 0;
}

int Solver::ship_tails() {
    if (multi()) {
        DS_CHECK(make_tails());
        DS_CHECK(group_begin());
        DS_CHECK(send_phi_head());
        DS_CHECK(send_tails());
        DS_CHECK(group_end());
    }
    return 0;
}

KktCoef Solver::kkt_coef() const {
    KktCoef k;
    k.sigma = sigma;
    k.kappa = sigma * cScale * D;
    k.dsD = dScale / D;
    k.dsE = dScale / E;
    return k;
}

int Solver::phase_q(int part, bool kkt) {
    if (!(fused && qrhs)) DS_CHECK(flush_alpha());
    prof_begin(PH_QSTEP);
    FOR_SLABS(s) {
        hipStream_t st = s.st;
        if (!fused) {
            DS_CHECK(launch_qstep(s.g, lc, s.phi, s.z, s.beta, s.weight, s.tail_bx, s.tail_by, s.q, s.alpha, s.st));
        } else {
            if (qrhs) {
                const i64 C = qstep_rhs_chunks(s.g, s.fg);
                i64 z0 = 0, zc = C, zs = 1;
                if (part == 1) { zc = C - 1; }
                else if (part == 2) { z0 = C - 1; zc = 1; }
                QStepExtra ex{};
                ex.apend = apend ? 1 : 0; ex.amul = amul; ex.adiv = adiv;
                if (multi() && !s.g.last && part != 1) ex.u0_tail = s.send_plane;
                if (kkt) {
                    const KktCoef k = kkt_coef();
                    ex.partials = kkt_qstep_partials(s.g, s.kw);
                    ex.resid = s.w1;
                    ex.kappa = k.kappa; ex.dsD = k.dsD;
                }
                DS_CHECK(launch_qstep_rhs(s.g, lc, s.fg, s.phi, s.q2, s.sx, s.sy, s.weight, s.tail_bx, s.tail_by, s.c,
                                          s.q_old, s.alpha, s.alpha2, s.w0, st, z0, zc, zs, &ex));
                if (part != 1) std::swap(s.alpha, s.alpha2);
            } else {
                DS_CHECK(launch_qstep_fused(s.g, lc, s.fg, s.phi, s.q2, s.sx, s.sy, s.weight, s.tail_bx, s.tail_by,
                                            s.q_old, s.alpha, s.st));
            }
            if (part != 1) std::swap(s.q, s.q_old);
        }
    }
    prof_end(PH_QSTEP);
    if (part == 1) return 0;
    u0_made = multi() && fused && qrhs;
    if (fused && qrhs) apend = false;
    rhs_valid = fused && qrhs;
    if (multi() && fused && comm_z && cone_split_enabled()) halo_pending = true;
    else DS_CHECK(exchange_q_halo(true));
    return 0;
}

int Solver::phase_mult() {
    if (fused) {
        deferred = true;
        return 0;
    }
    prof_begin(PH_BETA);
    FOR_SLABS(s) DS_CHECK(launch_beta_update(s.g, lc, s.q, s.z, s.beta, s.st));
    prof_end(PH_BETA);
    return 0;
}

int Solver::materialise() {
    if (!fused || !deferred) return 0;
    DS_CHECK(ensure_halo());
    prof_begin(PH_MATERIALISE);
    FOR_SLABS(s) {
        FusedArgs a{};
        a.q_old = s.q_old;
        a.q = s.q;
        a.beta_in = s.beta;
        a.beta_out = s.beta;
        a.z_out = s.z;
        set_pending(a);
        DS_CHECK(launch_cone_fused(2, s.g, lc, s.fg, a, s.st));
    }
    prof_end(PH_MATERIALISE);
    bpend = 0;
    deferred = false;
    z_valid = true;
    return 0;
}

int Solver::ensure_z() {
    if (!fused || z_valid) return 0;
    if (deferred) return materialise();
    if (!z_prev_ok) {
        set_error("internal: z cannot be regenerated");
        return DOTSOCP_ESTATE;
    }
    DS_CHECK(ensure_halo());
    prof_begin(PH_MATERIALISE);
    FOR_SLABS(s) {
        FusedArgs a{};
        a.q_old = s.q_old;
        a.q = s.q;
        a.beta_in = s.beta2;
        a.z_out = s.z;
        a.bpend = zp_pend;
        a.bmul = zp_mul; a.bdiv = zp_div; a.bmul2 = zp_mul2; a.bdiv2 = zp_div2;
        DS_CHECK(launch_cone_fused(3, s.g, lc, s.fg, a, s.st));
    }
    prof_end(PH_MATERIALISE);
    z_valid = true;
    return 0;
}

int Solver::kkt_sums(double *S, bool folded) {
    DS_CHECK(ensure_halo());
    const KktCoef k = kkt_coef();
    if (method == DOTSOCP_METHOD_ACCADMM && folded) {
        FOR_SLABS(s) DS_CHECK(launch_kkt_nodual(s.g, lc, k, s.phi, s.q, s.alpha, s.c, s.weight, s.kw, s.st));
        return reduce_sums(S);
    }
    if (!folded) {
        DS_CHECK(flush_alpha());
        FOR_SLABS(s)
            DS_HIP(ds_memset_async(s.kw.partials, 0, sizeof(double) * s.kw.maxBlocks * S_COUNT, s.st));
    }
    int rest = folded ? 0 : (1 | 4 | 8);
    if (fused && deferred) {
        FOR_SLABS(s) {
            FusedArgs a{};
            a.q_old = s.q_old;
            a.q = s.q;
            a.beta_in = s.beta;
            a.beta_out = s.beta2;
            set_pending(a);
            if (folded) { a.q2 = s.q2; a.sx = s.sx; a.sy = s.sy; }
            DS_CHECK(launch_kkt_cells_update(s.g, lc, k, s.fg, a, s.phi, s.alpha, s.weight, s.kw, s.st, folded, s.q));
            std::swap(s.beta, s.beta2);
        }
        zp_pend = bpend; zp_mul = bmul; zp_div = bdiv; zp_mul2 = bmul2; zp_div2 = bdiv2;
        bpend = 0;
        deferred = false;
        z_valid = false;
        z_prev_ok = true;
    } else {
        if (folded) { set_error("internal: folded KKT sums without a pending multiplier step"); return DOTSOCP_ESTATE; }
        DS_CHECK(ensure_z());
        DS_CHECK(flush_beta());
        rest |= 2;
    }
    if (multi()) {
        const i64 plane = slabs[0].g.plane;
        u0_made = false;
        FOR_SLABS(s)
            if (!s.g.last)
                DS_CHECK(launch_kkt_tail(s.g, s.alpha, s.beta, s.weight, s.send_plane, s.send_plane2, s.send_bx, s.send_by,
                                         s.st));
        DS_CHECK(group_begin());
        DS_CHECK(shift(+1, [](Slab &s) { return s.send_plane; }, [](Slab &s) { return s.a0_prev; }, plane));
        DS_CHECK(shift(+1, [](Slab &s) { return s.send_plane2; }, [](Slab &s) { return s.a0w_prev; }, plane));
        DS_CHECK(shift(+1, [](Slab &s) { return s.send_bx; }, [](Slab &s) { return s.btail_bx; }, slabs[0].g.bxLayer));
        DS_CHECK(shift(+1, [](Slab &s) { return s.send_by; }, [](Slab &s) { return s.btail_by; }, slabs[0].g.byLayer));
        DS_CHECK(group_end());
    }
    FOR_SLABS(s) {
        KktHalo halo{s.a0_prev, s.a0w_prev, s.btail_bx, s.btail_by};
        if (rest) DS_CHECK(launch_kkt(s.g, lc, k, s.phi, s.q, s.alpha, s.z, s.beta, s.c, s.weight, halo, s.kw, rest, s.st));
        if (folded && !s.g.first)
            DS_CHECK(launch_kkt(s.g, lc, k, s.phi, s.q, s.alpha, s.z, s.beta, s.c, s.weight, halo, s.kw, 1 | 4 | 8, s.st, true,
                                s.w1));
    }
    return reduce_sums(S);
}

int Solver::reduce_sums(double *S) {
    for (int i = 0; i <= S_COUNT; ++i) S[i] = 0.0;
    FOR_SLABS(s) {
        DS_CHECK(launch_kkt_final(s.g, s.kw, s.st));
        if (remote()) break;
        DS_HIP(ds_memcpy_async(s.h_sums, s.kw.sums, sizeof(double) * S_COUNT, hipMemcpyDeviceToHost, s.st));
    }
    if (!remote()) {
        FOR_SLABS(s) {
            DS_HIP(ds_stream_synchronize(s.st));
            for (int i = 0; i < S_COUNT; ++i) S[i] += s.h_sums[i];
        }
    }
    S[S_COUNT] = elapsed();
    if (remote()) {
        Rccl &api = rccl_api();
        Slab &s = slabs[0];
        DS_CHECK(comm_enter());
        const hipStream_t cs = cst(s);
        DS_NCCL(api.AllReduce(s.kw.sums, d_red, S_COUNT, ncclDouble, ncclSum, (ncclComm_t)nccl, cs));
        h_sums[S_COUNT] = S[S_COUNT];
        DS_HIP(ds_memcpy_async(d_red + S_COUNT, h_sums + S_COUNT, sizeof(double), hipMemcpyHostToDevice, cs));
        DS_NCCL(api.AllReduce(d_red + S_COUNT, d_red + S_COUNT, 1, ncclDouble, ncclMax, (ncclComm_t)nccl, cs));
        DS_HIP(ds_memcpy_async(h_sums, d_red, sizeof(double) * (S_COUNT + 1), hipMemcpyDeviceToHost, cs));
        DS_CHECK(comm_leave());
        DS_HIP(ds_stream_synchronize(stream));
        for (int i = 0; i <= S_COUNT; ++i) S[i] = h_sums[i];
    }
    elapsed_agreed = S[S_COUNT];
    return 0;
}

int Solver::norms_light(double *S) {
    DS_CHECK(ensure_halo());
    DS_CHECK(flush_alpha());
    const KktCoef k = kkt_coef();
    FOR_SLABS(s) {
        DS_HIP(ds_memset_async(s.kw.partials, 0, sizeof(double) * s.kw.maxBlocks * S_COUNT, s.st));
        FusedArgs a{};
        a.q_old = s.q_old;
        a.q = s.q;
        a.beta_in = s.beta;
        set_pending(a);
        DS_CHECK(launch_norms(s.g, lc, k, s.fg, a, s.phi, s.alpha, s.weight, s.kw, s.st));
    }
    return reduce_sums(S);
}

int Solver::rescale_block() {
    bool scaleYes = false;
    double normPhis = 0, normAlps = 0;
    auto norms = [&](double &nPhis, double &nAlps) -> int {
        double S[S_COUNT + 1];
        double sig = sigma;
        if (method == DOTSOCP_METHOD_INPALM && fused && last_S_it == it - 1 && norm_cache) {
            for (int i = 0; i < S_COUNT; ++i) S[i] = last_S[i];
            sig = last_S_sigma;
        } else if (method == DOTSOCP_METHOD_INPALM && fused && deferred && norm_cache) {
            DS_CHECK(norms_light(S));
        } else {
            DS_CHECK(materialise());
            DS_CHECK(ensure_z());
            DS_CHECK(kkt_sums(S));
        }
        const double sh = sqrt(h);
        const double normPhi = sh * sqrt(S[S_PHI2]), normQ = sh * sqrt(S[S_Q2]), normZ = sh * sqrt(S[S_Z2]);
        const double normAlpha = sig * (sh * sqrt(S[S_ALPHA2])), normBeta = sig * (sh * sqrt(S[S_BETA2]));
        nPhis = std::max(std::max(normPhi, normQ), normZ);
        nAlps = std::max(normAlpha, normBeta);
        return 0;
    };
    if (rescale >= 3 && (it % 100) == 0) {
        DS_CHECK(norms(normPhis, normAlps));
        const double ratio = std::max(normAlps, normPhis) / std::min(normAlps, normPhis);
        if (ratio > 1.2) scaleYes = true;
    }
    const bool first = (rescale == 1) && (maxFeas < 2e-2) && (it >= 10) && (relGap < 5e-2);
    const bool second = (rescale == 2) && (maxFeas < 5e-3) && (it >= 50) && (relGap < 1e-2);
    if (!(first || second || scaleYes)) return 0;
    if (!scaleYes) DS_CHECK(norms(normPhis, normAlps));
    DS_CHECK(materialise());
    const double dScale2 = normPhis, cScale2 = normAlps;
    sigma = sigma * (cScale2 / dScale2);
    norm_c = norm_c / cScale2;
    if (!prob.weighted) norm_d = norm_d / dScale2;
    DS_CHECK(scale_state(dScale2, cScale2 * cScale2, dScale2, true));
    if (method == DOTSOCP_METHOD_PALM) {
        FOR_SLABS(s) DS_CHECK(launch_scale(s.phi, s.g.NphiAlloc, 1.0, dScale2, s.st));
    }
    dScale = dScale2 * dScale;
    cScale = cScale2 * cScale;
    sigmaScale = sigmaScale * (cScale2 / dScale2);
    update_coef();
    rescale += 1;
    return 0;
}

bool if_adjust_sigma(double iter, double last_iter) {
    const double passed = iter - last_iter;
    if (iter < 20 && passed >= 3) return true;
    if (iter < 50 && passed >= 6) return true;
    if (iter < 100 && passed >= 10) return true;
    if (iter < 200 && passed >= 15) return true;
    if (iter < 500 && passed >= 25) return true;
    return passed >= 40;
}

static const double kUpdateRule[11][2] = {
    {1.1, 1.10}, {1.2, 1.15}, {1.5, 1.20}, {2, 1.26}, {2.5, 1.28}, {3.33, 1.32},
    {5, 1.35}, {10, 1.40}, {20, 1.60}, {40, 1.80}, {50, 2.00}};

static double get_factor(double xi) {
    double factor = 1.0;
    for (int i = 0; i < 11; ++i) {
        if (xi >= kUpdateRule[i][0]) factor = kUpdateRule[i][1];
        else break;
    }
    return factor;
}

static void adjust_lagrangian_param(double &sigma, double xi, double &factor) {
    factor = 1.0;
    if (xi >= 1) factor = get_factor(xi);
    else if (xi < 1) factor = 1.0 / get_factor(1.0 / xi);
    if (factor != 1.0) {
        const double old = sigma;
        sigma = std::max(std::min(sigma * factor, 1e3), 1e-3);
        factor = sigma / old;
    }
}

int Solver::kkt_block(bool adjustSigmaYes, bool timed_out, bool *brk, bool folded) {
    double S[S_COUNT + 1];
    prof_begin(PH_KKT);
    DS_CHECK(kkt_sums(S, folded));
    prof_end(PH_KKT);
    if (remote()) timed_out = elapsed_agreed > time_limit;
    for (int i = 0; i < S_COUNT; ++i) last_S[i] = S[i];
    last_S_sigma = sigma;
    last_S_it = it;
    const double sh = sqrt(h);
    auto nrm = [&](int i) { return sh * sqrt(S[i]); };
    const double norm_q = nrm(S_Q2), norm_z = nrm(S_Z2), norm_Aphi = nrm(S_APHI2);
    const double norm_alpha = sigma * nrm(S_ALPHA2), norm_beta = sigma * nrm(S_BETA2);
    const double norm_FBbeta = sigma * nrm(S_FBBETA2);
    const double primFea1 = nrm(S_PRIM1), primFea2 = nrm(S_PRIM2);
    const double dualFea1 = sigma * nrm(S_DUAL1), dualFea2 = sigma * nrm(S_DUAL2);
    const double complem = nrm(S_COMPLEM);
    const double dotcomplem = nrm(S_DOTCOMP), normRho = nrm(S_RHO2), norm_rhoFq = nrm(S_RHOFQ2);
    const double mRhoB = nrm(S_MRHOB), normM = nrm(S_M2), normRhoB = nrm(S_RHOB2);
    const double kc = 1.0;
    const double den2 = prob.weighted ? (norm_q + norm_z) : norm_d;
    double org[7], res[5];
    org[0] = primFea1 / (kc * D / dScale + norm_Aphi + norm_q);
    org[1] = primFea2 / (kc * E / dScale + den2);
    org[2] = dualFea1 / (kc / cScale + norm_c);
    org[3] = complem / (kc * E / dScale + norm_z + norm_beta);
    org[4] = dualFea2 / (kc / cScale / D + norm_FBbeta + norm_alpha);
    org[5] = dotcomplem / (kc + normRho + norm_rhoFq);
    org[6] = mRhoB / (kc + normM + normRhoB);
    res[0] = primFea1 / (kc + norm_Aphi + norm_q);
    res[1] = primFea2 / (kc + den2);
    res[2] = dualFea1 / (kc + norm_c);
    res[3] = complem / (kc + norm_z + norm_beta);
    res[4] = dualFea2 / (kc + norm_FBbeta + norm_alpha);
    const double priVal = (sigma * cScale * dScale * h) * S[S_QALPHA];
    const double dualVal = (sigma * cScale * dScale * h) * S[S_CPHI];
    const double pdGap = fabs(priVal - dualVal) / (1 + fabs(priVal) + fabs(dualVal));
    for (int i = 0; i < 7; ++i) hist_kkt.push_back(org[i]);
    hist_time.push_back(remote() ? elapsed_agreed : elapsed());
    hist_iter.push_back((double)it);
    hist_gap.push_back(pdGap);
    double mstop = std::max(std::max(org[0], org[2]), org[5]);
    if (checkPrimDualFeas) mstop = std::max(mstop, org[6]);
    if (mstop < opts.tol || timed_out) {
        *brk = true;
        return 0;
    }
    const double maxRes = *std::max_element(res, res + 5);
    if (maxRes < tol_feasOrg) use_feasOrg = 1;
    if (adjustSigmaYes) {
        lastSigmaIt = (double)it;
        double resiPri, resiDual;
        if (use_feasOrg) { resiPri = std::max(org[0], org[1]); resiDual = std::max(org[2], org[4]); }
        else { resiPri = std::max(res[0], res[1]); resiDual = std::max(res[2], res[4]); }
        double factor;
        adjust_lagrangian_param(sigma, resiPri / resiDual, factor);
        if (factor != 1.0) {
            if (folded && rhs_valid && method != DOTSOCP_METHOD_ACCADMM) DS_CHECK(sigma_scale_folded(factor));
            else DS_CHECK(scale_state(1.0, factor, 1.0, true));
            if (method == DOTSOCP_METHOD_ACCADMM) DS_CHECK(acc_on_sigma_factor(factor));
        }
    }
    if (rescale > 0) {
        maxFeas = maxRes;
        relGap = pdGap;
    }
    return 0;
}

int Solver::step(bool *brk) {
    *brk = false;
    if (method == DOTSOCP_METHOD_ACCADMM) return acc_step(brk);
    if (method == DOTSOCP_METHOD_PALM) return palm_step(brk);
    it += 1;
    DS_CHECK(rescale_block());
    const bool adjustSigmaYes = if_adjust_sigma((double)it, lastSigmaIt);
    const bool kkt_due = opts.ifCheckStepByStep || adjustSigmaYes || it == opts.maxit;
    const bool fold = kkt_due && kkt_fold && fused && qrhs;
    const bool inter = comm_z && multi() && fused && qrhs;
    bool split = inter && cone_split_enabled();
    for (auto &s : slabs) split = split && s.fg.chunks >= 2;
    bool split_q = inter && cone_split_enabled();
    for (auto &s : slabs) split_q = split_q && qstep_rhs_chunks(s.g, s.fg) >= 2;
    auto async_comm = [&](const std::function<int()> &fn, hipEvent_t Slab::*ev) -> int {
        DS_CHECK(comm_fork());
        comm_async = true;
        const int rc = fn();
        comm_async = false;
        DS_CHECK(rc);
        return comm_mark(ev);
    };
    if (inter) {
        const bool pend = halo_pending;
        if (pend) {
            DS_CHECK(make_u0_tail());
            DS_CHECK(async_comm([&]() { return ensure_halo(); }, &Slab::ev_halo));
        }
        if (split) DS_CHECK(phase_z(1));
        if (pend) DS_CHECK(comm_wait(&Slab::ev_halo));
        if (!split) DS_CHECK(phase_z(0));
        PhiHooks hooks;
        hooks.fill = [&]() -> int {
            if (split) DS_CHECK(phase_z(2));
            return make_tails();
        };
        hooks.behind = [&]() -> int { return async_comm([&]() { return send_tails(); }, &Slab::ev_join); };
        DS_CHECK(phase_phi(&hooks));
    } else {
        DS_CHECK(phase_phi());
        DS_CHECK(phase_z(0));
    }
    if (fold) {
        FOR_SLABS(s) DS_HIP(ds_memset_async(s.kw.partials, 0, sizeof(double) * s.kw.maxBlocks * S_COUNT, s.st));
    }
    if (inter) {
        DS_CHECK(async_comm([&]() { return send_phi_head(); }, &Slab::ev_halo));
        DS_CHECK(comm_wait(&Slab::ev_join));
        if (split_q) DS_CHECK(phase_q(1, fold));
        DS_CHECK(comm_wait(&Slab::ev_halo));
        DS_CHECK(phase_q(split_q ? 2 : 0, fold));
    } else {
        DS_CHECK(phase_z_tails());
        DS_CHECK(phase_q(0, fold));
    }
    DS_CHECK(phase_mult());
    const bool timed_out = remote() ? false : (elapsed() > time_limit);
    if (kkt_due || timed_out)
        DS_CHECK(kkt_block(adjustSigmaYes, timed_out, brk, fold));
    return 0;
}

int Solver::run(i64 n_iters, i64 *done) {
    if (!begun || finished) { set_error("run() needs begin() and must precede finish()"); return DOTSOCP_ESTATE; }
    cur_dev = -1;
    DS_CHECK(use_dev(device));
    struct DeferScope {
        DeferCtx *ctx;
        int err = 0;
        explicit DeferScope(DeferCtx *c) : ctx(c) { if (ctx) { g_defer = ctx; ctx->begin(); } }
        int close() { if (ctx) { err = ctx->end(); g_defer = nullptr; ctx = nullptr; } return err; }
        ~DeferScope() { (void)close(); }
    } scope(defer.get());
    i64 n = 0;
    while (it < opts.maxit && !stopped) {
        if (n_iters >= 0 && n >= n_iters) break;
        bool brk = false;
        DS_CHECK(step(&brk));
        if (brk) stopped = true;
        ++n;
    }
    DS_CHECK(ensure_halo());
    DS_CHECK(sync_all());
    DS_CHECK(prof_flush());
    if (const int derr = scope.close()) {
        set_error("a HIP call issued by a slab thread failed: %s", hipGetErrorString((hipError_t)derr));
        return DOTSOCP_EHIP;
    }
    if (done) *done = n;
    return 0;
}

int Solver::finish(dotsocp_result *res) {
    if (!begun) { set_error("finish() before begin()"); return DOTSOCP_ESTATE; }
    cur_dev = -1;
    DS_CHECK(use_dev(device));
    DS_CHECK(ensure_z());
    DS_CHECK(flush_beta());
    DS_CHECK(flush_alpha());
    DS_CHECK(sync_all());
    DS_CHECK(prof_flush());
    if (canary_enabled()) {
        std::string rep;
        const int bad = canary_check(&rep);
        cur_dev = -1;
        if (bad) {
            set_error("canary: %d device buffer(s) written out of bounds: %s", bad, rep.c_str());
            return DOTSOCP_EHIP;
        }
    }
    finished = true;
    if (res) {
        memset(res, 0, sizeof *res);
        res->sigma = sigma / sigmaScale;
        res->sigma_internal = sigma;
        res->cScale = cScale;
        res->dScale = dScale;
        res->times[0] = (phase_ms[PH_RHS] + phase_ms[PH_POISSON]) * 1e-3;
        res->times[1] = (phase_ms[PH_PROJ] + phase_ms[PH_FUSED_A] + phase_ms[PH_FUSED_B]) * 1e-3;
        res->times[2] = phase_ms[PH_QSTEP] * 1e-3;
        res->times[3] = (phase_ms[PH_BETA] + phase_ms[PH_MATERIALISE]) * 1e-3;
        res->times[4] = phase_ms[PH_KKT] * 1e-3;
        res->times[5] = elapsed();
        res->times[6] = (double)it;
        res->iters = it;
        res->hist_len = (i64)hist_iter.size();
        res->stopped = stopped ? 1 : 0;
        if (method == DOTSOCP_METHOD_PALM) res->time_extra = phase_ms[PH_QSTEP0] * 1e-3;
        if (method == DOTSOCP_METHOD_ACCADMM) {
            res->times[0] = (phase_ms[PH_RHS] + phase_ms[PH_POISSON]) * 1e-3;
            res->times[1] = phase_ms[PH_ACC_CONE] * 1e-3;
            res->times[2] = (phase_ms[PH_QSTEP] + phase_ms[PH_ACC_GATHER]) * 1e-3;
            res->times[3] = 0.0;
            res->time_extra = phase_ms[PH_INTERP] * 1e-3;
        }
    }
    return 0;
}

}
```

dot-socp_amd/csrc/solver_io.hip:

```cpp
#include <algorithm>
#include <cstring>

#include "solver.h"

namespace dotsocp {

int Solver::recover_outputs(const double *rho0, const double *rho1, double *rho, double *Ex, double *Ey, double *q0,
                            double *bx, double *by) {
    if (!finished) { set_error("recover_outputs() needs finish()"); return DOTSOCP_ESTATE; }
    DS_ARG(rho == nullptr || (rho0 != nullptr && rho1 != nullptr), "rho needs rho0 and rho1");
    cur_dev = -1;
    DS_CHECK(use_dev(device));
    const i64 plane = slabs[0].g.plane;
    const i64 hplane = ny * nx;
    const i64 py = slabs[0].g.py;
    const double cD = cScale * D, dD = dScale / D;
    if (rho && multi()) {
        FOR_SLABS(s)
            if (!s.g.last) DS_CHECK(launch_out_tail(s.g, s.alpha, s.weight, sigma, cD, s.send_plane, s.st));
        DS_CHECK(shift(+1, [](Slab &s) { return s.send_plane; }, [](Slab &s) { return s.a0_prev; }, plane));
    }
    double *outs[6] = {rho, Ex, Ey, q0, bx, by};
    for (int which = 0; which < 6; ++which) {
        if (!outs[which]) continue;
        {
            i64 layers = 0;
            for (auto &s : slabs) layers += (which >= 3) ? s.g.ncl : s.g.ntl;
            host_first_touch(outs[which], sizeof(double) * (size_t)(hplane * layers));
        }
        FOR_SLABS(s) {
            const Grid &g = s.g;
            double *d_r0 = s.w1, *d_r1 = s.w1 + plane;
            if (which == 0) {
                if (g.first) DS_CHECK(copy_rows(d_r0, const_cast<double *>(rho0), ny, py, nx, true, s.st));
                if (g.last) DS_CHECK(copy_rows(d_r1, const_cast<double *>(rho1), ny, py, nx, true, s.st));
            }
            const i64 layers = (which >= 3) ? g.ncl : g.ntl;
            DS_CHECK(launch_outputs(g, s.q, s.alpha, s.weight, d_r0, d_r1, s.a0_prev, sigma, cD, dD, which, s.w0, s.st));
            double *h = outs[which] + (remote() ? 0 : hplane * g.t0);
            if (layers > 0) DS_CHECK(copy_rows(s.w0, h, ny, py, nx * layers, false, s.st));
        }
        DS_CHECK(sync_all());
    }
    return 0;
}

int Solver::jump_from(Solver &coarse) {
    if (begun) { set_error("jump_next_level() must precede begin() of the fine level"); return DOTSOCP_ESTATE; }
    if (!coarse.finished) { set_error("jump_next_level() needs finish() of the coarse level"); return DOTSOCP_ESTATE; }
    DS_ARG(!remote() && !coarse.remote(), "multilevel transfer between one-slab-per-process contexts goes through the host");
    DS_ARG(prob.dim == coarse.prob.dim && prob.weighted == coarse.prob.weighted, "level kinds differ");
    DS_ARG(ny == 2 * (coarse.ny - 1) + 1 && nt == 2 * (coarse.nt - 1) + 1 &&
               (nx == 2 * (coarse.nx - 1) + 1 || (nx == 1 && coarse.nx == 1)),
           "fine grid must be 2 (n - 1) + 1 of the coarse grid in every dimension");
    cur_dev = -1;
    DS_CHECK(use_dev(device));
    DS_CHECK(ensure_alloc());
    coarse.cur_dev = -1;
    DS_CHECK(coarse.sync_all());
    cur_dev = -1;
    cScale = prob.cScale; dScale = prob.dScale; D = prob.D; E = prob.E;
    update_coef();
    const i64 planec = coarse.slabs[0].g.plane;
    auto pull = [&](Slab &f, double *dst, const Slab &c, const double *src, i64 count) -> int {
        if (count <= 0) return 0;
        const size_t bytes = sizeof(double) * (size_t)count;
        if (f.dev == c.dev) DS_HIP(ds_memcpy_async(dst, src, bytes, hipMemcpyDeviceToDevice, f.st));
        else DS_HIP(ds_memcpy_peer_async(dst, f.dev, src, c.dev, bytes, f.st));
        return 0;
    };
    const bool direct = !multi() && !coarse.multi() && slabs[0].dev == coarse.slabs[0].dev;
    FOR_SLABS(f) {
        const Grid &gf = f.g;
        const Grid &gc0 = coarse.slabs[0].g;
        if (direct) {
            Slab &c = coarse.slabs[0];
            DS_CHECK(launch_prolong_phi(gf, c.g, c.phi, f.phi, coarse.dScale, 1.0 / dScale, f.st));
            DS_CHECK(launch_prolong_beta(gf, c.g, c.beta, f.beta, f.z, coarse.sigma, coarse.cScale * coarse.E,
                                         1.0 / cScale / E, f.st));
            continue;
        }
        const i64 tlast = gf.t0 + gf.ntl - 1;
        const i64 nA = gf.t0 >> 1, nB = (tlast >> 1) + (tlast & 1);
        for (auto &c : coarse.slabs) {
            const i64 a = std::max<i64>(nA, c.g.t0), b = std::min<i64>(nB, c.g.t0 + c.g.ntl - 1);
            if (a <= b) DS_CHECK(pull(f, f.w0 + planec * (a - nA), c, c.phi + planec * (a - c.g.t0), planec * (b - a + 1)));
        }
        DS_CHECK(launch_prolong_phi(gf, gc0, f.w0, f.phi, coarse.dScale, 1.0 / dScale, f.st, nA));
        if (gf.ncl > 0) {
            const i64 cA = gf.t0 >> 1, cB = (gf.t0 + gf.ncl - 1) >> 1, nl = cB - cA + 1;
            double *tmp = f.beta2;
            if (!tmp) { set_error("multilevel transfer on time slabs needs the fused dataflow"); return DOTSOCP_EINVAL; }
// ... 44 lines not shown
```

dot-socp_amd/csrc/stencil.hip:

```cpp
#include "device_utils.h"
#include "kernels.h"

#include <cstdlib>

namespace dotsocp {

static inline dim3 tile_grid(const Grid &g, i64 layers) {
    return dim3((unsigned)((g.ny + TILE_Y - 1) / TILE_Y), (unsigned)((g.nx + TILE_X - 1) / TILE_X), (unsigned)layers);
}

template <bool WEIGHTED>
__global__ void __launch_bounds__(TILE_Y *TILE_X) k_rhs(RhsArgs a, double *__restrict__ rhs) {
    const i64 y = (i64)blockIdx.x * TILE_Y + threadIdx.x;
    const i64 x = (i64)blockIdx.y * TILE_X + threadIdx.y;
    const i64 tl = blockIdx.z;
    if (y >= a.g.ny || x >= a.g.nx) return;
    rhs[y + a.g.py * (x + a.g.nx * tl)] = rhs_value<WEIGHTED>(a, y, x, tl);
}

int launch_rhs(const Grid &g, const LoopCoef &c, const double *q, const double *alpha, const double *cvec,
               const double *weight, const double *u0_prev, double *rhs, hipStream_t st) {
    if (g.Nphi <= 0) return 0;
    RhsArgs a{g, c.at, c.ax, c.ay, q, alpha, cvec, weight, u0_prev};
    if (weight)
        DS_KLAUNCH(k_rhs<true>, tile_grid(g, g.ntl), dim3(TILE_Y, TILE_X), 0, st, a, rhs);
    else
        DS_KLAUNCH(k_rhs<false>, tile_grid(g, g.ntl), dim3(TILE_Y, TILE_X), 0, st, a, rhs);
    DS_HIP(hipGetLastError());
    return 0;
}

template <bool WEIGHTED>
__global__ void __launch_bounds__(TILE_Y *TILE_X) k_u0_tail(Grid g, const double *__restrict__ q,
                                                             const double *__restrict__ alpha,
                                                             const double *__restrict__ weight,
                                                             double *__restrict__ out) {
    const i64 y = (i64)blockIdx.x * TILE_Y + threadIdx.x;
    const i64 x = (i64)blockIdx.y * TILE_X + threadIdx.y;
    if (y >= g.ny || x >= g.nx) return;
    const i64 k = y + g.py * (x + g.nx * (g.ncl - 1));
    out[y + g.py * x] = WEIGHTED ? weight[k] * q[k] - alpha[k] : q[k] - alpha[k];
}

int launch_u0_tail(const Grid &g, const double *q, const double *alpha, const double *weight, double *out,
                   hipStream_t st) {
    if (g.ncl <= 0) return 0;
    if (weight)
        DS_KLAUNCH(k_u0_tail<true>, tile_grid(g, 1), dim3(TILE_Y, TILE_X), 0, st, g, q, alpha, weight, out);
    else
        DS_KLAUNCH(k_u0_tail<false>, tile_grid(g, 1), dim3(TILE_Y, TILE_X), 0, st, g, q, alpha, weight, out);
    DS_HIP(hipGetLastError());
    return 0;
}

struct WSum {
    const double *z, *b;
    i64 Nz;
    __device__ __forceinline__ double operator()(int j, i64 cell) const { return z[j * Nz + cell] + b[j * Nz + cell]; }
};

template <bool WEIGHTED, int VAR = 0>
__device__ __forceinline__ void q_update(const LoopCoef &c, double tmp, double q2, double diag_c, double dinv, i64 k,
                                         const double *__restrict__ weight, double *__restrict__ q,
                                         double *alpha, const double *alpha_in = nullptr) {
    const double a = (VAR == 1) ? alpha_in[k] : alpha[k];
    double qn, r;
    if (WEIGHTED) {
        const double w = weight[k];
        const double di = 1.0 / (diag_c + w * w);
        qn = (w * (tmp + a) + q2) * di;
        r = tmp - w * qn;
    } else {
        qn = (tmp + a + q2) * dinv;
        r = tmp - qn;
    }
    q[k] = qn;
    if (VAR == 2) return;
    if (VAR == 1) {
        const double t = a + tmp;
        alpha[k] = WEIGHTED ? t - weight[k] * qn : t - qn;
    } else {
        alpha[k] = a + c.tau * r;
    }
}

template <bool WEIGHTED, int SEG>
__global__ void __launch_bounds__(TILE_Y *TILE_X) k_qstep(Grid g, LoopCoef c, const double *__restrict__ phi,
                                                           const double *__restrict__ z,
                                                           const double *__restrict__ beta,
                                                           const double *__restrict__ weight,
                                                           const double *__restrict__ tail_bx,
                                                           const double *__restrict__ tail_by,
                                                           double *__restrict__ q, double *__restrict__ alpha) {
    const i64 y = (i64)blockIdx.x * TILE_Y + threadIdx.x;
    const i64 x = (i64)blockIdx.y * TILE_X + threadIdx.y;
    const i64 tl = blockIdx.z;
    WSum W{z, beta, g.Nc};
    const i64 node = y + g.py * (x + g.nx * tl);
    if (SEG == 0) {
        if (y >= g.ny || x >= g.nx) return;
        double tmp = (-c.at) * phi[node];
        tmp += c.at * phi[node + g.plane];
        const double q2 = c.s * (W(9, node) - W(0, node));
        q_update<WEIGHTED>(c, tmp, q2, c.c1, c.dinv1, node, weight, q, alpha);
    } else {
        const bool tbnd = (g.t0 + tl == 0) || (g.t0 + tl == g.nt - 1);
// ... 155 lines not shown
        } else if (MULT == 1) {
            const double t = a + tmp;
            an = t - w * qn;
        } else {
            const double r = tmp - w * qn;
            an = a + c.tau * r;
        }
        u = w * qn - an;
    } else {
        qn = (tmp + a + q2) * dinv;
        if (MULT == 2) {
            an = a;
        } else if (MULT == 1) {
            const double t = a + tmp;
            an = t - qn;
        } else {
            const double r = tmp - qn;
            an = a + c.tau * r;
        }
        u = qn - an;
    }
    return a;
}

template <bool WEIGHTED, int MULT = 0>
__device__ __forceinline__ double q_calc(const LoopCoef &c, double tmp, double q2, double diag_c, double dinv, double w,
                                         double a, const APend &ap, double &qn, double &an, double &u) {
    if (ap.on) a = a * ap.mul / ap.div;
    if (WEIGHTED) {
        const double di = 1.0 / (diag_c + w * w);
        qn = (w * (tmp + a) + q2) * di;
        if (MULT == 2) {
            an = a;
        } else if (MULT == 1) {
            const double t = a + tmp;
            an = t - w * qn;
        } else {
            const double r = tmp - w * qn;
            an = a + c.tau * r;
        }
        u = w * qn - an;
    } else {
        qn = (tmp + a + q2) * dinv;
        if (MULT == 2) {
            an = a;
        } else if (MULT == 1) {
            const double t = a + tmp;
            an = t - qn;
        } else {
            const double r = tmp - qn;
            an = a + c.tau * r;
        }
        u = qn - an;
    }
    return a;
}

__device__ __forceinline__ double fbbf_cell(const LoopCoef &c, double q0) {
    return c.s * ((c.dF + c.s * q0) - (c.dF - c.s * q0));
}
__device__ __forceinline__ double fbbf_edge(const LoopCoef &c, double e, bool tbnd) {
    const double v = c.sf * e;
    double acc = v + v;
    if (!tbnd) {
        acc += v;
        acc += v;
    }
    return c.sf * acc;
}

struct QRhsArgs {
    const double *phi, *q2v, *sx, *sy, *weight, *tail_bx, *tail_by, *cvec, *alpha_in;
    double *q_out, *alpha_out, *rhs;
    double *u0_tail;
    i64 TC, z0, zstride;
    double *q_state;
    const double *q_anchor, *alpha_anchor;
    double c1, c2, om_rho, rho;
    APend ap;
    int xcd;
    const double *qk;
    double *partials, *resid;
    double kappa, dsD;
};

enum { Q_Q2 = 0, Q_ALPHA2, Q_APHI2, Q_PRIM1, Q_QALPHA, Q_CPHI, Q_PHI2, Q_DUAL1, Q_MRHOB, Q_M2, Q_RHOB2, Q_COUNT };

template <bool WEIGHTED, int VAR, bool KKT = false, int QTX = TILE_X>
__global__ void __launch_bounds__(TILE_Y *QTX, (QTX > TILE_X && !WEIGHTED ? 4 : 1)) k_qstep_rhs(Grid g, LoopCoef c, FusedGeom fg, QRhsArgs a) {
    __shared__ double xch[2][QTX][TILE_Y];
    __shared__ double ph[2][QTX + 2][TILE_Y + 2];
    __shared__ double xcha[KKT ? 2 : 1][KKT ? QTX : 1][KKT ? TILE_Y : 1];
    __shared__ double xchr[KKT ? 2 : 1][KKT ? QTX : 1][KKT ? TILE_Y : 1];
    double S[Q_COUNT];
    if (KKT) {
#pragma unroll
        for (int i = 0; i < Q_COUNT; ++i) S[i] = 0.0;
    }
    auto wgt = [&](i64 k) { return WEIGHTED ? a.weight[k] : 1.0; };
    auto entry = [&](double tmp, double qn, double an, double w) {
        const double wq = w * qn;
        S[Q_Q2] += qn * qn;
        S[Q_ALPHA2] += an * an;
        S[Q_APHI2] += tmp * tmp;
        const double r1 = tmp - wq;
        S[Q_PRIM1] += r1 * r1;
        S[Q_QALPHA] += wq * an;
    };
    double a0prev = 0.0, rhoTprev = 0.0;
    const int lane = threadIdx.x, xl = threadIdx.y;
    const BlockId blk = block_id(a.xcd != 0);
    const i64 y = (i64)blk.x * TILE_Y + lane;
    const i64 x = (i64)blk.y * QTX + xl;
    const bool inb = (y < g.ny) && (x < g.nx);
    const i64 t0 = ((i64)blk.z * a.zstride + a.z0) * a.TC;
    const i64 t1 = (t0 + a.TC < g.ntl) ? t0 + a.TC : g.ntl;
    auto put = [&](i64 k, double qn, double an, double ain) {
        a.q_out[k] = qn;
        if (VAR == 3) return;
        if (VAR == 2) {
            double t = a.om_rho * a.q_state[k];
            t = t + a.rho * qn;
            a.q_state[k] = a.c1 * a.q_anchor[k] + a.c2 * t;
            t = a.om_rho * ain;
            t = t + a.rho * an;
            a.alpha_out[k] = a.c1 * a.alpha_anchor[k] + a.c2 * t;
        } else {
            a.alpha_out[k] = an;
        }
    };
    double u0prev = 0.0;
    double p0 = 0.0;
    const bool hasBx0 = inb && (x < g.nx - 1), hasBy0 = inb && (y < g.ny - 1);
    const bool rightCol = hasBx0 && (xl == QTX - 1), topRow = hasBy0 && (lane == TILE_Y - 1);
    if (inb) {
        const i64 node0 = y + g.py * (x + g.nx * t0);
        p0 = a.phi[node0];
        double hx = 0.0, hl = 0.0, hy = 0.0, hb = 0.0;
        if (rightCol) hx = a.phi[node0 + g.py];
        if (xl == 0 && x >= 1) hl = a.phi[node0 - g.py];
        if (topRow) hy = a.phi[node0 + 1];
        if (lane == 0 && y >= 1) hb = a.phi[node0 - 1];
        ph[0][xl + 1][lane + 1] = p0;
        if (xl == QTX - 1) ph[0][QTX + 1][lane + 1] = hx;
        if (xl == 0) ph[0][0][lane + 1] = hl;
        if (lane == TILE_Y - 1) ph[0][xl + 1][TILE_Y + 1] = hy;
        if (lane == 0) ph[0][xl + 1][0] = hb;
        if (t0 > 0) {
            const i64 k = node0 - g.plane;
            double tmp = (-c.at) * a.phi[k];
            tmp += c.at * p0;
            double qn, an;
            double g0f = a.q2v[k];
            if (VAR == 3 && a.qk) g0f = g0f - c.tau * fbbf_cell(c, a.qk[k]);
            q_value<WEIGHTED, (VAR == 3 ? 2 : (VAR != 0 ? 1 : 0))>(c, tmp, g0f, c.c1, c.dinv1, k, a.weight, a.alpha_in, qn, an, u0prev, a.ap);
            if (KKT) {
                a0prev = an;
                rhoTprev = a.kappa * (wgt(k) * an);
            }
        }
    }
    constexpr int MULT = (VAR == 3 ? 2 : (VAR != 0 ? 1 : 0));
    const i64 yc = inb ? y : 0, xc = inb ? x : 0;
    const bool hasBx = inb && (x < g.nx - 1), hasBy = inb && (y < g.ny - 1);
    const bool leftTile = inb && (xl == 0) && (x >= 1);
    const bool belowTile = inb && (lane == 0) && (y >= 1);
    const bool sxOwn = hasBx && ((x % fg.XB) == fg.XB - 1), syOwn = hasBy && ((y & 63) == 63);
    int par = 0;
    __syncthreads();
    for (i64 tl = t0; tl < t1; ++tl) {
        const i64 node = yc + g.py * (xc + g.nx * tl);
        const bool tbnd = (g.t0 + tl == 0) || (g.t0 + tl == g.nt - 1);
        const double dc = tbnd ? c.c2 : c.c1;
        const double di = tbnd ? c.dinv2 : c.dinv1;
        const bool hasCell = inb && (tl < g.ncl);
        const bool tails = (tl == 0) && !g.first;
        const bool lay0 = KKT && tails;
        const i64 eX = hasBx ? g.offBx + g.bxLayer * tl + yc + g.py * xc : node;
        const i64 eY = hasBy ? g.offBy + g.byLayer * tl + yc + g.pyb * xc : node;
        const i64 k0 = hasCell ? node : 0;
        const i64 nodeT = hasCell ? node + g.plane : node;
        const double pTl = a.phi[nodeT];
        double hx = 0.0, hl = 0.0, hy = 0.0, hb = 0.0;
        if (rightCol) hx = a.phi[nodeT + g.py];
        if (leftTile) hl = a.phi[nodeT - g.py];
        if (topRow) hy = a.phi[nodeT + 1];
        if (belowTile) hb = a.phi[nodeT - 1];
        const double pXl = ph[par][xl + 2][lane + 1];
        const double pYl = ph[par][xl + 1][lane + 2];
        const double al0 = a.alpha_in[k0], alX = a.alpha_in[eX], alY = a.alpha_in[eY];
        double g0 = a.q2v[k0];
        double gX = a.q2v[eX], gY = a.q2v[eY];
        double k0v = 0.0, kXv = 0.0, kYv = 0.0;
        const bool pcorr = (VAR == 3) && (a.qk != nullptr);
        if (pcorr) { k0v = a.qk[k0]; kXv = a.qk[eX]; kYv = a.qk[eY]; }
        const double cv = a.cvec[node];
        double w0 = 1.0, wX = 1.0, wY = 1.0;
        if (WEIGHTED) { w0 = a.weight[k0]; wX = a.weight[eX]; wY = a.weight[eY]; }
        const double sxv = a.sx[sxOwn ? (tl * fg.nxblk + (x / fg.XB + 1)) * g.ny + y : 0];
        const double syv = a.sy[syOwn ? (tl * g.nx + x) * fg.nyblk + (y / 64 + 1) : 0];
        double tXv = 0.0, tYv = 0.0;
        if (tails) {
            if (hasBx) tXv = a.tail_bx[y + g.py * x];
            if (hasBy) tYv = a.tail_by[y + g.pyb * x];
        }
        double pLl = 0.0, alL = 0.0, gL = 0.0, wL = 1.0, sxL = 0.0, tLv = 0.0, kLv = 0.0, kBv = 0.0;
        i64 eL = 0;
        if (leftTile) {
            eL = g.offBx + g.bxLayer * tl + y + g.py * (x - 1);
            pLl = ph[par][0][lane + 1];
            alL = a.alpha_in[eL];
            gL = a.q2v[eL];
            if (pcorr) kLv = a.qk[eL];
            if (WEIGHTED) wL = a.weight[eL];
            if (((x - 1) % fg.XB) == fg.XB - 1) sxL = a.sx[(tl * fg.nxblk + ((x - 1) / fg.XB + 1)) * g.ny + y];
            if (tails) tLv = a.tail_bx[y + g.py * (x - 1)];
        }
        double pBl = 0.0, alB = 0.0, gB = 0.0, wB = 1.0, syB = 0.0, tBv = 0.0;
        i64 eB = 0;
        if (belowTile) {
            eB = g.offBy + g.byLayer * tl + (y - 1) + g.pyb * x;
            pBl = ph[par][xl + 1][0];
            alB = a.alpha_in[eB];
            gB = a.q2v[eB];
            if (pcorr) kBv = a.qk[eB];
            if (WEIGHTED) wB = a.weight[eB];
            if (((y - 1) & 63) == 63) syB = a.sy[(tl * g.nx + x) * fg.nyblk + ((y - 1) / 64 + 1)];
            if (tails) tBv = a.tail_by[(y - 1) + g.pyb * x];
        }
        if (sxOwn) gX = c.sf * (gX + sxv);
        if (syOwn) gY = c.sf * (gY + syv);
        if (tails) { gX += tXv; gY += tYv; }
        if (pcorr) {
            g0 = g0 - c.tau * fbbf_cell(c, k0v);
            gX = gX - c.tau * fbbf_edge(c, kXv, tbnd);
            gY = gY - c.tau * fbbf_edge(c, kYv, tbnd);
        }
        double pT = 0.0, u0 = 0.0, ubx = 0.0, uby = 0.0;
        double a0 = 0.0, abx = 0.0, aby = 0.0;
        double qbx = 0.0, mbx = 0.0, qby = 0.0, mby = 0.0;
        double rhoT = 0.0;
        double q0n = 0.0, a0n = 0.0, ain0 = 0.0, qXn = 0.0, aXn = 0.0, ainX = 0.0, qYn = 0.0, aYn = 0.0, ainY = 0.0;
        if (hasCell) {
            pT = pTl;
            double tmp = (-c.at) * p0;
            tmp += c.at * pT;
            ain0 = q_calc<WEIGHTED, MULT>(c, tmp, g0, c.c1, c.dinv1, w0, al0, a.ap, q0n, a0n, u0);
            if (KKT) {
                entry(tmp, q0n, a0n, w0);
                a0 = a0n;
                rhoT = a.kappa * (w0 * a0n);
            }
        }
        if (hasBx) {
            double tmp = (-c.ax) * p0;
            tmp += c.ax * pXl;
            ainX = q_calc<WEIGHTED, MULT>(c, tmp, gX, dc, di, wX, alX, a.ap, qXn, aXn, ubx);
            if (KKT) {
                abx = aXn;
                qbx = qXn;
                if (!lay0) {
                    entry(tmp, qXn, aXn, wX);
                    mbx = a.kappa * (wX * aXn);
                    S[Q_M2] += mbx * mbx;
                }
            }
        }
        if (hasBy) {
            double tmp = (-c.ay) * p0;
            tmp += c.ay * pYl;
            ainY = q_calc<WEIGHTED, MULT>(c, tmp, gY, dc, di, wY, alY, a.ap, qYn, aYn, uby);
            if (KKT) {
                aby = aYn;
                qby = qYn;
                if (!lay0) {
                    entry(tmp, qYn, aYn, wY);
                    mby = a.kappa * (wY * aYn);
                    S[Q_M2] += mby * mby;
                }
// ... 67 lines not shown
            if (y <= g.ny - 2) r += (-c.ay) * uby;
            a.rhs[node] = r + cv;
            if (KKT && !lay0) {
                double ra = 0.0;
                if (tl >= 1) ra += c.at * a0prev;
                if (tl < g.ncl) ra += (-c.at) * a0;
                if (x >= 1) ra += c.ax * abx_m;
                if (x <= g.nx - 2) ra += (-c.ax) * abx;
                if (y >= 1) ra += c.ay * aby_m;
                if (y <= g.ny - 2) ra += (-c.ay) * aby;
                ra = ra - cv;
                a.resid[node] = ra;
                S[Q_DUAL1] += ra * ra;
                S[Q_CPHI] += cv * p0;
                S[Q_PHI2] += p0 * p0;
                if (x < g.nx - 1 && xl < QTX - 1) {
                    const double rm = (rhoN + xchr[par][xl + 1][lane]) / 2.0;
                    const double rb = a.dsD * (rm * qbx);
                    const double d = mbx - rb;
                    S[Q_MRHOB] += d * d;
                    S[Q_RHOB2] += rb * rb;
                }
                if (y < g.ny - 1 && lane < TILE_Y - 1) {
                    const double rm = (rhoN + rhoU) / 2.0;
                    const double rb = a.dsD * (rm * qby);
                    const double d = mby - rb;
                    S[Q_MRHOB] += d * d;
                    S[Q_RHOB2] += rb * rb;
                }
            }
        }
        u0prev = u0;
        if (KKT) {
            a0prev = a0;
            rhoTprev = rhoT;
        }
        p0 = pT;
        par ^= 1;
    }
    if (KKT) {
        __shared__ double red[QTX][Q_COUNT];
        static const int slot[Q_COUNT] = {S_Q2, S_ALPHA2, S_APHI2, S_PRIM1, S_QALPHA, S_CPHI, S_PHI2, S_DUAL1, S_MRHOB, S_M2, S_RHOB2};
#pragma unroll
        for (int i = 0; i < Q_COUNT; ++i) {
            double v = S[i];
#pragma unroll
            for (int off = 32; off >= 1; off >>= 1) v += __shfl_down(v, off, 64);
            if (lane == 0) red[xl][i] = v;
        }
        __syncthreads();
        if (xl == 0 && lane < S_COUNT) {
            double v = 0.0;
#pragma unroll
            for (int i = 0; i < Q_COUNT; ++i)
                if (slot[i] == lane) {
                    v = red[0][i];
#pragma unroll
                    for (int wv = 1; wv < QTX; ++wv) v += red[wv][i];
                }
            const i64 b = blk.x + (i64)gridDim.x * (blk.y + (i64)gridDim.y * ((i64)blk.z * a.zstride + a.z0));
            a.partials[b * S_COUNT + lane] = v;
        }
    }
}

static int launch_qstep_rhs_var(int var, const Grid &g, const LoopCoef &c, const FusedGeom &fg, QRhsArgs a, hipStream_t st,
                                i64 z0 = 0, i64 zcount = -1, i64 zstride = 1);

int launch_qstep_rhs(const Grid &g, const LoopCoef &c, const FusedGeom &fg, const double *phi, const double *q2,
                     const double *sx, const double *sy, const double *weight, const double *tail_bx,
                     const double *tail_by, const double *cvec, double *q_out, const double *alpha_in, double *alpha_out,
                     double *rhs, hipStream_t st, i64 z0, i64 zcount, i64 zstride, const QStepExtra *ex) {
    QRhsArgs a{};
    a.phi = phi; a.q2v = q2; a.sx = sx; a.sy = sy; a.weight = weight; a.tail_bx = tail_bx; a.tail_by = tail_by;
    a.cvec = cvec; a.alpha_in = alpha_in; a.q_out = q_out; a.alpha_out = alpha_out; a.rhs = rhs;
    a.ap = APend{0, 1.0, 1.0};
    if (ex) {
        a.ap = APend{ex->apend, ex->amul, ex->adiv};
        a.partials = ex->partials;
        a.resid = ex->resid;
        a.u0_tail = ex->u0_tail;
        a.kappa = ex->kappa;
        a.dsD = ex->dsD;
    }
    return launch_qstep_rhs_var(0, g, c, fg, a, st, z0, zcount, zstride);
}

i64 qstep_rhs_blocks(const Grid &g, const FusedGeom &fg) { return fg.nyblk * fg.nxblk * qstep_rhs_chunks(g, fg); }

__global__ void __launch_bounds__(256) k_rhs_sigma_fix(double *__restrict__ rhs, const double *__restrict__ r,
                                                        double *__restrict__ cvec, i64 n, double factor) {
    for (i64 i = (i64)blockIdx.x * blockDim.x + threadIdx.x; i < n; i += (i64)gridDim.x * blockDim.x) {
        const double rv = r[i];
        rhs[i] = (rhs[i] + rv) - rv / factor;
        cvec[i] = cvec[i] / factor;
    }
}

int launch_rhs_sigma_fix(double *rhs, const double *r, double *cvec, i64 n, double factor, hipStream_t st) {
    if (n <= 0) return 0;
    DS_KLAUNCH(k_rhs_sigma_fix, dim3(launch_blocks(n, 256, 1 << 22)), dim3(256), 0, st, rhs, r, cvec, n, factor);
    DS_HIP(hipGetLastError());
    return 0;
}

int launch_qstep_rhs_acc(int var, const Grid &g, const LoopCoef &c, const FusedGeom &fg, const double *phi,
                         const double *q2, const double *sx, const double *sy, const double *weight, const double *cvec,
                         double *q_raw, const double *alpha_in, double *alpha_out, double *rhs, double *q_state,
                         const double *q_anchor, const double *alpha_anchor, const AccCoef &k, hipStream_t st,
                         const double *tail_bx, const double *tail_by, double *u0_tail) {
    QRhsArgs a{};
    a.phi = phi; a.q2v = q2; a.sx = sx; a.sy = sy; a.weight = weight; a.cvec = cvec;
    a.tail_bx = tail_bx; a.tail_by = tail_by; a.u0_tail = u0_tail;
    a.alpha_in = alpha_in; a.q_out = q_raw; a.alpha_out = alpha_out; a.rhs = rhs;
    a.q_state = q_state; a.q_anchor = q_anchor; a.alpha_anchor = alpha_anchor;
    a.c1 = k.c1; a.c2 = k.c2; a.om_rho = k.om_rho; a.rho = k.rho;
    return launch_qstep_rhs_var(var, g, c, fg, a, st);
}

i64 qstep_rhs_chunks(const Grid &g, const FusedGeom &fg, i64 *TCout) {
    const i64 tiles = fg.nyblk * fg.nxblk;
    const i64 target = 32768;
    i64 chunks = (target + tiles - 1) / tiles;
    i64 TC = (g.ntl + chunks - 1) / chunks;
    if (TC < 8) TC = 8;
    if (!(g.first && g.last) && cone_split_enabled() && g.ntl >= 12) {
        const i64 tail = (g.ntl / 4 < 4) ? 4 : g.ntl / 4;
        const i64 body = g.ntl - tail, nb = (body + 7) / 8;
        TC = (body + nb - 1) / nb;
    }
    if (TC > g.ntl) TC = g.ntl;
    if (TC < 1) TC = 1;
    if (TCout) *TCout = TC;
    return (g.ntl + TC - 1) / TC;
}

static int launch_qstep_rhs_var(int var, const Grid &g, const LoopCoef &c, const FusedGeom &fg, QRhsArgs a, hipStream_t st,
                                i64 z0, i64 zcount, i64 zstride) {
    i64 TC = 1;
    const i64 chunks = qstep_rhs_chunks(g, fg, &TC);
    if (zcount < 0) zcount = chunks - z0;
    if (z0 < 0 || zcount <= 0 || zstride < 1 || z0 + (zcount - 1) * zstride >= chunks) return 0;
    a.TC = TC;
    a.z0 = z0;
    a.zstride = zstride;
    a.xcd = 1;
    dim3 grid((unsigned)fg.nyblk, (unsigned)fg.nxblk, (unsigned)zcount);
    dim3 blk(TILE_Y, TILE_X);
    const char *qe = getenv("DOTSOCP_QTX");
    const int qtx_env = qe ? atoi(qe) : 0;
    const int qtx = qtx_env ? qtx_env : ((fg.nyblk * fg.nxblk * zcount >= 8192 && !a.weight) ? 2 * TILE_X : TILE_X);
    if (var == 0 && !a.partials && qtx == 2 * TILE_X) {
        dim3 grid2((unsigned)fg.nyblk, (unsigned)((g.nx + 2 * TILE_X - 1) / (2 * TILE_X)), (unsigned)zcount);
        dim3 blk2(TILE_Y, 2 * TILE_X);
        if (a.weight) DS_KLAUNCH((k_qstep_rhs<true, 0, false, 2 * TILE_X>), grid2, blk2, 0, st, g, c, fg, a);
        else DS_KLAUNCH((k_qstep_rhs<false, 0, false, 2 * TILE_X>), grid2, blk2, 0, st, g, c, fg, a);
        DS_HIP(hipGetLastError());
        return 0;
    }
#define QRHS_LAUNCH(W, V) DS_KLAUNCH((k_qstep_rhs<W, V>), grid, blk, 0, st, g, c, fg, a)
    if (var == 0 && a.partials) {
        if (a.weight) DS_KLAUNCH((k_qstep_rhs<true, 0, true>), grid, blk, 0, st, g, c, fg, a);
        else DS_KLAUNCH((k_qstep_rhs<false, 0, true>), grid, blk, 0, st, g, c, fg, a);
    } else if (a.weight) {
        if (var == 0) QRHS_LAUNCH(true, 0); else if (var == 1) QRHS_LAUNCH(true, 1); else QRHS_LAUNCH(true, 2);
    } else {
        if (var == 0) QRHS_LAUNCH(false, 0); else if (var == 1) QRHS_LAUNCH(false, 1);
        else if (var == 2) QRHS_LAUNCH(false, 2); else QRHS_LAUNCH(false, 3);
    }
#undef QRHS_LAUNCH
    DS_HIP(hipGetLastError());
    return 0;
}

__global__ void __launch_bounds__(TILE_Y *TILE_X) k_rhs_fixup(Grid g, double at, const double *__restrict__ u0_prev,
                                                               double *__restrict__ rhs) {
    const i64 y = (i64)blockIdx.x * TILE_Y + threadIdx.x;
    const i64 x = (i64)blockIdx.y * TILE_X + threadIdx.y;
    if (y >= g.ny || x >= g.nx) return;
    const i64 i = y + g.py * x;
    rhs[i] = rhs[i] + at * u0_prev[i];
}

int launch_rhs_fixup(const Grid &g, const LoopCoef &c, const double *u0_prev, double *rhs, hipStream_t st) {
// ... 150 lines not shown
```

include/dotsocp.h:

```cpp
#ifndef DOTSOCP_H
#define DOTSOCP_H

#ifdef __cplusplus
extern "C" {
#endif

typedef long long dotsocp_i64;

enum {
    DOTSOCP_OK = 0,
    DOTSOCP_EINVAL = -1,
    DOTSOCP_ENODEVICE = -2,
    DOTSOCP_EHIP = -3,
    DOTSOCP_ESTATE = -4,
    DOTSOCP_ECOMM = -5
};

const char *dotsocp_last_error(void);
const char *dotsocp_version(void);
int dotsocp_device_count(void);
dotsocp_i64 dotsocp_release_cache(void);


int dotsocp_proj_soc(double *out, const double *in, dotsocp_i64 M, dotsocp_i64 K);
// ... 8 lines not shown

int dotsocp_bfd_conj1d(double *q, const double *z, dotsocp_i64 nt, dotsocp_i64 nx, double scale);

int dotsocp_oper_poisson(double *res, const double *rhs, dotsocp_i64 ny, dotsocp_i64 nx,
                         dotsocp_i64 nt, double kernelScale);

int dotsocp_dctn(double *a, dotsocp_i64 ny, dotsocp_i64 nx, dotsocp_i64 nt, int inverse);

int dotsocp_proj_soc_dev(double *d_out, const double *d_in, dotsocp_i64 M, dotsocp_i64 K, void *stream);
int dotsocp_bfd_dev(double *d_z, const double *d_q, dotsocp_i64 nt, dotsocp_i64 nx, dotsocp_i64 ny,
                    double scale, double dF, void *stream);
int dotsocp_bfd_conj_dev(double *d_q, const double *d_z, dotsocp_i64 nt, dotsocp_i64 nx, dotsocp_i64 ny,
                         double scale, void *stream);


typedef struct dotsocp_ctx dotsocp_ctx;

typedef struct {
    int dim;
    int weighted;
    dotsocp_i64 ny, nx, nt;
    double D, E;
    double cScale, dScale;
    double normc, normd;
} dotsocp_problem;

typedef struct {
    double tau;
    double sigma;
    double tol;
    dotsocp_i64 maxit;
    int ifCheckStepByStep;
    int checkPrimDualFeas;
    int scaling;
    double time_limit;
} dotsocp_opts;

enum {
    DOTSOCP_METHOD_INPALM = 0,
    DOTSOCP_METHOD_PALM = 1,
    DOTSOCP_METHOD_ACCADMM = 2
};

typedef struct {
    dotsocp_i64 restart;
    double rho;
    double theta;
} dotsocp_acc_opts;

enum {
    DOTSOCP_F_PHI = 0,
    DOTSOCP_F_Q = 1,
    DOTSOCP_F_ALPHA = 2,
    DOTSOCP_F_Z = 3,
    DOTSOCP_F_BETA = 4,
    DOTSOCP_F_C = 5,
    DOTSOCP_F_WEIGHT = 6
};

typedef struct {
    double sigma;
    double sigma_internal;
    double cScale, dScale;
    double times[7];
    dotsocp_i64 iters;
    dotsocp_i64 hist_len;
    int stopped;
    double time_extra;
} dotsocp_result;

dotsocp_ctx *dotsocp_create(const dotsocp_problem *prob, int device, int nslabs);
dotsocp_ctx *dotsocp_create_multi(const dotsocp_problem *prob, int first_device, int ngpu);
void dotsocp_destroy(dotsocp_ctx *ctx);

int dotsocp_rccl_unique_id(unsigned char id[128]);
int dotsocp_attach_rccl(dotsocp_ctx *ctx, const unsigned char id[128], int rank, int world);

int dotsocp_slab_range(dotsocp_i64 nt, int world, int rank, dotsocp_i64 *t0, dotsocp_i64 *t1);

dotsocp_i64 dotsocp_field_len(const dotsocp_problem *prob, int field);

int dotsocp_dct_algorithm(dotsocp_i64 n);

int dotsocp_upload(dotsocp_ctx *ctx, int field, const double *host);
int dotsocp_download(dotsocp_ctx *ctx, int field, double *host);
int dotsocp_upload_layers(dotsocp_ctx *ctx, int field, const double *host, dotsocp_i64 t0, dotsocp_i64 n);

int dotsocp_begin(dotsocp_ctx *ctx, const dotsocp_opts *opts);
int dotsocp_begin_method(dotsocp_ctx *ctx, const dotsocp_opts *opts, int method, const dotsocp_acc_opts *acc);
int dotsocp_run(dotsocp_ctx *ctx, dotsocp_i64 n_iters, dotsocp_i64 *done);
int dotsocp_finish(dotsocp_ctx *ctx, dotsocp_result *res);

int dotsocp_recover_outputs(dotsocp_ctx *ctx, const double *rho0, const double *rho1, double *rho, double *Ex,
                            double *Ey, double *q0, double *bx, double *by);

int dotsocp_jump_next_level(dotsocp_ctx *coarse, dotsocp_ctx *fine);

int dotsocp_get_history(dotsocp_ctx *ctx, double *kkt, double *time, double *iter, double *pdGap);

int dotsocp_set_profiling(dotsocp_ctx *ctx, int on);
int dotsocp_kernel_time(dotsocp_ctx *ctx, const char *name, double *avg_ms, dotsocp_i64 *launches);

int dotsocp_canary_check(void);

int dotsocp_synchronize(dotsocp_ctx *ctx);

#ifdef __cplusplus
}
#endif
#endif
```

Measured before the change: 81.31.

## Carry beta in gamma form across fused cone passes and skip zero interior c reads

Splits the beta multiplier update into a carry term (beta + tau*z) written by one MODE_B cone pass and a finish term (gamma - tau*v) applied by the next. This lets the following pass skip reloading q_old and rebuilding/projecting z whenever no KKT check, sigma update, rescale or end of run needs real beta. It also detects at begin time whether c is zero away from the first and last time layers and, if so, skips interior c reads in the RHS kernels and the sigma fix. The cost is extra state, guards that refuse any path that meets the gamma form, and deferred timeout handling.

```diff
diff --git a/dot-socp_amd/capi.py b/dot-socp_amd/capi.py
--- a/dot-socp_amd/capi.py
+++ b/dot-socp_amd/capi.py
@@ -67,6 +67,8 @@
     "dotsocp_slab_range": (ctypes.c_int, [i64, ctypes.c_int, ctypes.c_int, ctypes.POINTER(i64), ctypes.POINTER(i64)]),
     "dotsocp_field_len": (i64, [ctypes.POINTER(Problem), ctypes.c_int]),
     "dotsocp_dct_algorithm": (ctypes.c_int, [i64]),
+    "dotsocp_cone_writes_beta": (ctypes.c_int, [i64, dbl, i64, ctypes.c_int, ctypes.c_int, ctypes.c_int, dbl, dbl]),
+    "dotsocp_rescale_due": (ctypes.c_int, [i64, ctypes.c_int, dbl, dbl]),
     "dotsocp_release_cache": (i64, []),
     "dotsocp_upload": (ctypes.c_int, [vp, ctypes.c_int, vp]),
     "dotsocp_upload_layers": (ctypes.c_int, [vp, ctypes.c_int, vp, i64, i64]),
diff --git a/dot-socp_amd/csrc/capi.hip b/dot-socp_amd/csrc/capi.hip
--- a/dot-socp_amd/csrc/capi.hip
+++ b/dot-socp_amd/csrc/capi.hip
@@ -277,6 +277,14 @@
 
 int dotsocp_dct_algorithm(dotsocp_i64 n) { return dct_choose_algorithm(n); }
 
+int dotsocp_cone_writes_beta(dotsocp_i64 it, double last_sigma_it, dotsocp_i64 maxit, int check_step_by_step,
+                             int last_of_run, int rescale, double maxFeas, double relGap) {
+    return cone_writes_beta(it, last_sigma_it, maxit, check_step_by_step != 0, last_of_run != 0, rescale, maxFeas, relGap) ? 1 : 0;
+}
+int dotsocp_rescale_due(dotsocp_i64 it, int rescale, double maxFeas, double relGap) {
+    return rescale_due(it, rescale, maxFeas, relGap) ? 1 : 0;
+}
+
 dotsocp_i64 dotsocp_field_len(const dotsocp_problem *p, int field) {
     if (!p || (p->dim != 1 && p->dim != 2) || p->nt < 2 || p->nx < 1 || (p->dim == 2 && p->ny < 1)) return -1;
     const i64 ny = p->dim == 1 ? p->nx : p->ny, nx = p->dim == 1 ? 1 : p->nx, nt = p->nt;
@@ -343,7 +351,7 @@
     DS_ARG(name != nullptr, "name is NULL");
     static const char *names[PH_COUNT] = {"rhs", "poisson", "cone_proj", "qstep", "beta", "kkt",
                                           "cone_fused_a", "cone_fused_b", "materialise", "comm",
-                                          "interp", "acc_cone", "acc_gather", "qstep_first", "transpose"};
+                                          "interp", "acc_cone", "acc_gather", "qstep_first", "transpose", "cone_carry"};
     for (int i = 0; i < PH_COUNT; ++i)
         if (strcmp(name, names[i]) == 0) {
             const i64 n = ctx->s.phase_launches[i];
diff --git a/dot-socp_amd/csrc/cone.hip b/dot-socp_amd/csrc/cone.hip
--- a/dot-socp_amd/csrc/cone.hip
+++ b/dot-socp_amd/csrc/cone.hip
@@ -136,10 +136,8 @@
             for (int j = 0; j < 10; ++j) zout[j * g.Nc + i] = v[j];
         } else {
 #pragma unroll
-            for (int j = 0; j < 10; ++j) {
-                const double r = zin[j * g.Nc + i] - v[j];
-                betaout[j * g.Nc + i] = betain[j * g.Nc + i] + c.tau * r;
-            }
+            for (int j = 0; j < 10; ++j)
+                betaout[j * g.Nc + i] = mult_finish(mult_carry(betain[j * g.Nc + i], zin[j * g.Nc + i], c.tau), v[j], c.tau);
         }
         cur = nxt;
     }
diff --git a/dot-socp_amd/csrc/device_utils.h b/dot-socp_amd/csrc/device_utils.h
--- a/dot-socp_amd/csrc/device_utils.h
+++ b/dot-socp_amd/csrc/device_utils.h
@@ -70,6 +70,9 @@
     for (int j = 1; j < K; ++j) v[j] = c * v[j];
     v[0] = (c >= 1.0) ? v[0] : c * n;
 }
+
+__device__ __forceinline__ double mult_carry(double b, double z, double tau) { return fma(tau, z, b); }
+__device__ __forceinline__ double mult_finish(double g, double v, double tau) { return fma(-tau, v, g); }
 
 struct EdgeQuad {
     double xm, xp, ym, yp;
@@ -145,6 +148,7 @@
     Grid g;
     double at, ax, ay;
     const double *q, *alpha, *cvec, *weight, *u0_prev;
+    int c_ends;
 };
 
 template <bool WEIGHTED>
@@ -164,7 +168,9 @@
     const i64 byo = g.offBy + g.byLayer * tl;
     if (y >= 1) r += a.ay * u(byo + (y - 1) + g.pyb * x);
     if (y <= g.ny - 2) r += (-a.ay) * u(byo + y + g.pyb * x);
-    return r + a.cvec[node];
+    const bool tbnd = (g.t0 + tl == 0) || (g.t0 + tl == g.nt - 1);
+    const double cv = (a.c_ends && !tbnd) ? 0.0 : a.cvec[node];
+    return r + cv;
 }
 
 }
diff --git a/dot-socp_amd/csrc/fused.hip b/dot-socp_amd/csrc/fused.hip
--- a/dot-socp_amd/csrc/fused.hip
+++ b/dot-socp_amd/csrc/fused.hip
@@ -6,8 +6,9 @@
 
 namespace dotsocp {
 
-template <int MODE, int XB, bool NT = false>
+template <int MODE, int XB, bool NT = false, bool GIN = false, bool GOUT = false>
 __global__ void __launch_bounds__(64 * XB) k_cone_fused(Grid g, LoopCoef c, FusedArgs a) {
+    static_assert(MODE == 1 || !(GIN || GOUT), "the gamma form exists between two MODE_B passes only");
     constexpr bool DUAL = (MODE >= 5);
     constexpr bool UPD = (MODE != 0 && MODE != 6);
     constexpr bool PROJ = (MODE < 2 || MODE >= 5);
@@ -28,7 +29,7 @@
     const i64 nxblk = gridDim.y, nyblk = gridDim.x;
 
     EdgeQuad cur = load_edges(g, a.q, yc, xc, tstart, c.sf), curo, cur3;
-    if (UPD) curo = load_edges(g, a.q_old, yc, xc, tstart, c.sf);
+    if (UPD && !GIN) curo = load_edges(g, a.q_old, yc, xc, tstart, c.sf);
     if (MODE == 5) cur3 = load_edges(g, a.q3, yc, xc, tstart, c.sf);
     GatherCarry gc, gcp;
     if (carried) {
@@ -47,7 +48,7 @@
             double b[10], v[10];
 #pragma unroll
             for (int j = 0; j < 10; ++j) b[j] = ld_stream<NT>(a.beta_in + j * g.Nc + i);
-            if (a.bpend) {
+            if (!GIN && a.bpend) {
 #pragma unroll
                 for (int j = 0; j < 10; ++j) b[j] = b[j] * a.bmul / a.bdiv;
                 if (a.bpend > 1) {
@@ -56,7 +57,14 @@
                 }
             }
             build_z2(v, a.q[i], cur, nxt, c.s, c.dF);
-            if (UPD) {
+            if constexpr (GIN) {
+#pragma unroll
+                for (int j = 0; j < 10; ++j) b[j] = mult_finish(b[j], v[j], c.tau);
+                if (!GOUT && own && inb) {
+#pragma unroll
+                    for (int j = 0; j < 10; ++j) st_stream<NT>(a.beta_out + j * g.Nc + i, b[j]);
+                }
+            } else if constexpr (UPD) {
                 const EdgeQuad nxto = load_edges(g, a.q_old, yc, xc, tl + 1, c.sf);
                 double zo[10];
                 build_z2(zo, a.q_old[i], curo, nxto, c.s, c.dF);
@@ -64,12 +72,9 @@
                 for (int j = 0; j < 10; ++j) zo[j] = zo[j] - b[j];
                 proj_row<10>(zo);
 #pragma unroll
-                for (int j = 0; j < 10; ++j) {
-                    const double r = zo[j] - v[j];
-                    b[j] = b[j] + c.tau * r;
-                }
+                for (int j = 0; j < 10; ++j) b[j] = mult_finish(mult_carry(b[j], zo[j], c.tau), v[j], c.tau);
                 if (own && inb) {
-                    if (MODE != 3) {
+                    if (MODE != 3 && !GOUT) {
 #pragma unroll
                         for (int j = 0; j < 10; ++j) st_stream<NT>(a.beta_out + j * g.Nc + i, b[j]);
                     }
@@ -95,6 +100,10 @@
 #pragma unroll
                 for (int j = 0; j < 10; ++j) v[j] = v[j] - b[j];
                 proj_row<10>(v);
+                if (GOUT && own && inb) {
+#pragma unroll
+                    for (int j = 0; j < 10; ++j) st_stream<NT>(a.beta_out + j * g.Nc + i, mult_carry(b[j], v[j], c.tau));
+                }
 #pragma unroll
                 for (int j = 0; j < 10; ++j) w[j] = v[j] + b[j];
                 if (own && inb) a.q2[i] = c.s * (w[9] - w[0]);
@@ -164,7 +173,7 @@
 }
 
 int launch_cone_fused(int mode, const Grid &g, const LoopCoef &c, const FusedGeom &fg, FusedArgs a,
-                      hipStream_t st, i64 z0, i64 zcount) {
+                      hipStream_t st, i64 z0, i64 zcount, int flavour) {
     if (g.Nz <= 0) return 0;
     if (zcount < 0) zcount = fg.chunks - z0;
     if (z0 < 0 || zcount <= 0 || z0 + zcount > fg.chunks) return 0;
@@ -179,6 +188,19 @@
         if (nt) DS_KLAUNCH((k_cone_fused<M, 4, true>), grid, blk, 0, st, g, c, a);       \
         else DS_KLAUNCH((k_cone_fused<M, 4>), grid, blk, 0, st, g, c, a);                \
         break;
+    if (flavour != 0) {
+        if (mode != 1 || (flavour & ~(CONE_GIN | CONE_GOUT))) { set_error("bad fused flavour"); return DOTSOCP_EINVAL; }
+        if ((flavour & CONE_GIN) && a.bpend) { set_error("internal: gamma with a pending scaling"); return DOTSOCP_ESTATE; }
+#define CONE_FLAV(GI, GO)                                                                          \
+        if (nt) DS_KLAUNCH((k_cone_fused<1, 4, true, GI, GO>), grid, blk, 0, st, g, c, a);         \
+        else DS_KLAUNCH((k_cone_fused<1, 4, false, GI, GO>), grid, blk, 0, st, g, c, a);
+        if (flavour == CONE_GOUT) { CONE_FLAV(false, true) }
+        else if (flavour == CONE_GIN) { CONE_FLAV(true, false) }
+        else { CONE_FLAV(true, true) }
+#undef CONE_FLAV
+        DS_HIP(hipGetLastError());
+        return 0;
+    }
     switch (mode) {
         CONE_MODE(0) CONE_MODE(1) CONE_MODE(2) CONE_MODE(3) CONE_MODE(4) CONE_MODE(5) CONE_MODE(6)
 #undef CONE_MODE
diff --git a/dot-socp_amd/csrc/kernels.h b/dot-socp_amd/csrc/kernels.h
--- a/dot-socp_amd/csrc/kernels.h
+++ b/dot-socp_amd/csrc/kernels.h
@@ -65,8 +65,9 @@
 };
 bool tile_xcd_remap(const Grid &g);
 int fused_geometry(const Grid &g, FusedGeom &fg);
+enum { CONE_GIN = 1, CONE_GOUT = 2 };
 int launch_cone_fused(int mode, const Grid &g, const LoopCoef &c, const FusedGeom &fg, FusedArgs a,
-                      hipStream_t st, i64 z0 = 0, i64 zcount = -1);
+                      hipStream_t st, i64 z0 = 0, i64 zcount = -1, int flavour = 0);
 bool cone_split_enabled();
 
 struct KktWork;
@@ -117,6 +118,7 @@
     double *partials, *resid;
     double kappa, dsD;
     double *u0_tail;
+    int c_ends;
 };
 int launch_qstep_rhs(const Grid &g, const LoopCoef &c, const FusedGeom &fg, const double *phi, const double *q2,
                      const double *sx, const double *sy, const double *weight, const double *tail_bx,
@@ -124,7 +126,9 @@
                      double *rhs, hipStream_t st, i64 z0 = 0, i64 zcount = -1, i64 zstride = 1,
                      const QStepExtra *ex = nullptr);
 i64 qstep_rhs_blocks(const Grid &g, const FusedGeom &fg);
-int launch_rhs_sigma_fix(double *rhs, const double *r, double *cvec, i64 n, double factor, hipStream_t st);
+int launch_rhs_sigma_fix(const Grid &g, double *rhs, const double *r, double *cvec, double factor, hipStream_t st,
+                         bool c_ends = false);
+int launch_c_interior_test(const Grid &g, const double *cvec, int *flag, hipStream_t st);
 i64 qstep_rhs_chunks(const Grid &g, const FusedGeom &fg, i64 *TC = nullptr);
 int launch_qstep_rhs_acc(int var, const Grid &g, const LoopCoef &c, const FusedGeom &fg, const double *phi,
                          const double *q2, const double *sx, const double *sy, const double *weight, const double *cvec,
@@ -142,7 +146,7 @@
 int launch_kkt_tail(const Grid &g, const double *alpha, const double *beta, const double *weight, double *a0,
                     double *a0w, double *bt_bx, double *bt_by, hipStream_t st);
 int launch_rhs(const Grid &g, const LoopCoef &c, const double *q, const double *alpha, const double *cvec,
-               const double *weight, const double *u0_prev, double *rhs, hipStream_t st);
+               const double *weight, const double *u0_prev, double *rhs, hipStream_t st, bool c_ends = false);
 int launch_qstep(const Grid &g, const LoopCoef &c, const double *phi, const double *z, const double *beta,
                  const double *weight, const double *tail_bx, const double *tail_by, double *q,
                  double *alpha, hipStream_t st);
diff --git a/dot-socp_amd/csrc/kkt.hip b/dot-socp_amd/csrc/kkt.hip
--- a/dot-socp_amd/csrc/kkt.hip
+++ b/dot-socp_amd/csrc/kkt.hip
@@ -234,7 +234,7 @@
 #pragma unroll
                 for (int j = 0; j < 10; ++j) {
                     const double r = zo[j] - v[j];
-                    b[j] = b[j] + c.tau * r;
+                    b[j] = mult_finish(mult_carry(b[j], zo[j], c.tau), v[j], c.tau);
                     zs += zo[j] * zo[j];
                     bs += b[j] * b[j];
                     rs += r * r;
diff --git a/dot-socp_amd/csrc/solver.h b/dot-socp_amd/csrc/solver.h
--- a/dot-socp_amd/csrc/solver.h
+++ b/dot-socp_amd/csrc/solver.h
@@ -62,6 +62,7 @@
     double *z = nullptr;
     double *beta = nullptr;
     double *c = nullptr;
+    bool c_ends = false;
     double *weight = nullptr;
     double *w0 = nullptr, *w1 = nullptr;
     i64 l0 = 0, nl = 0;
@@ -87,7 +88,11 @@
 bool if_adjust_sigma(double iter, double last_iter);
 
 enum Phase { PH_RHS = 0, PH_POISSON, PH_PROJ, PH_QSTEP, PH_BETA, PH_KKT, PH_FUSED_A, PH_FUSED_B, PH_MATERIALISE,
-             PH_COMM, PH_INTERP, PH_ACC_CONE, PH_ACC_GATHER, PH_QSTEP0, PH_TRANSPOSE, PH_COUNT };
+             PH_COMM, PH_INTERP, PH_ACC_CONE, PH_ACC_GATHER, PH_QSTEP0, PH_TRANSPOSE, PH_CONE_CARRY, PH_COUNT };
+
+bool rescale_due(i64 it, int rescale, double maxFeas, double relGap);
+bool cone_writes_beta(i64 it, double lastSigmaIt, i64 maxit, bool checkStepByStep, bool last_of_run, int rescale,
+                      double maxFeas, double relGap);
 
 struct Solver {
     dotsocp_problem prob{};
@@ -153,6 +158,15 @@
     bool z_valid = true;
     bool z_prev_ok = false;
     int ensure_z();
+    bool cone_carry = true;
+    bool beta_gamma = false;
+    bool cone_gout = false;
+    bool last_of_run = false;
+    i64 timeout_at = -1;
+    bool timeout_pending = false;
+    int need_beta_form(const char *who) const;
+    bool c_ends_on = true;
+    int detect_c_ends();
     int bpend = 0;
     double bmul = 1.0, bdiv = 1.0, bmul2 = 1.0, bdiv2 = 1.0;
     int push_beta_op(double mul, double div);
diff --git a/dot-socp_amd/csrc/solver.hip b/dot-socp_amd/csrc/solver.hip
--- a/dot-socp_amd/csrc/solver.hip
+++ b/dot-socp_amd/csrc/solver.hip
@@ -961,6 +961,22 @@
     return copy_field(*this, field, const_cast<double *>(host), true);
 }
 
+int Solver::detect_c_ends() {
+    FOR_SLABS(s) {
+        int *flag = nullptr, h = 1;
+        DS_CHECK(dmalloc(&flag, 1));
+        int rc = 0;
+        if (ds_memset_async(flag, 0, sizeof(int), s.st) != hipSuccess) rc = DOTSOCP_EHIP;
+        if (!rc) rc = launch_c_interior_test(s.g, s.c, flag, s.st);
+        if (!rc && ds_memcpy_async(&h, flag, sizeof(int), hipMemcpyDeviceToHost, s.st) != hipSuccess) rc = DOTSOCP_EHIP;
+        if (!rc && ds_stream_synchronize(s.st) != hipSuccess) rc = DOTSOCP_EHIP;
+        dfree(flag);
+        if (rc) { if (rc == DOTSOCP_EHIP) set_error("the zero test of c failed"); return rc; }
+        s.c_ends = (h == 0);
+    }
+    return 0;
+}
+
 int Solver::upload_layers(int field, const double *host, i64 t0, i64 n) {
     DS_ARG(host != nullptr, "host pointer is NULL");
     DS_ARG(field == DOTSOCP_F_PHI || field == DOTSOCP_F_C, "layer uploads serve the node fields (phi, c)");
@@ -992,6 +1008,7 @@
     DS_CHECK(use_dev(device));
     DS_CHECK(ensure_alloc());
     if (field == DOTSOCP_F_Z || field == DOTSOCP_F_BETA) {
+        DS_CHECK(need_beta_form("download"));
         DS_CHECK(ensure_z());
         DS_CHECK(flush_beta());
     }
@@ -1066,7 +1083,14 @@
     lc.dinv2 = 1.0 / lc.c2;
 }
 
+int Solver::need_beta_form(const char *who) const {
+    if (!beta_gamma) return 0;
+    set_error("internal: %s met the gamma form of beta", who);
+    return DOTSOCP_ESTATE;
+}
+
 int Solver::flush_beta() {
+    DS_CHECK(need_beta_form("flush_beta"));
     if (!bpend) return 0;
     FOR_SLABS(s) {
         DS_CHECK(launch_scale(s.beta, 10 * s.g.Nc, bmul, bdiv, s.st));
@@ -1102,11 +1126,12 @@
         apend = true; amul = 1.0; adiv = factor;
     }
     u0_fresh = false;
-    FOR_SLABS(s) DS_CHECK(launch_rhs_sigma_fix(s.w0, s.w1, s.c, s.g.Nphi, factor, s.st));
+    FOR_SLABS(s) DS_CHECK(launch_rhs_sigma_fix(s.g, s.w0, s.w1, s.c, factor, s.st, c_ends_on && s.c_ends));
     return 0;
 }
 
 int Solver::scale_state(double a_mul, double a_div, double q_div, bool with_c) {
+    DS_CHECK(need_beta_form("scale_state"));
     DS_CHECK(flush_alpha());
     if (begun) DS_CHECK(ensure_halo());
     u0_made = false;
@@ -1154,6 +1179,17 @@
         fused = false;
     }
     opts = *o;
+    cone_carry = true;
+    if (const char *e = getenv("DOTSOCP_CONE_CARRY")) cone_carry = (atoi(e) != 0);
+    c_ends_on = true;
+    if (const char *e = getenv("DOTSOCP_C_ENDS")) c_ends_on = (atoi(e) != 0);
+    if (c_ends_on) DS_CHECK(detect_c_ends());
+    timeout_at = -1;
+    if (const char *e = getenv("DOTSOCP_TEST_TIMEOUT_AT")) timeout_at = atoll(e);
+    beta_gamma = false;
+    cone_gout = false;
+    last_of_run = false;
+    timeout_pending = false;
     checkPrimDualFeas = (o->checkPrimDualFeas < 0) ? !prob.weighted : (o->checkPrimDualFeas != 0);
     time_limit = (o->time_limit > 0) ? o->time_limit : 3600.0;
     sigma = o->sigma;
@@ -1254,7 +1290,7 @@
     prof_begin(PH_RHS);
     if (!rhs_valid) {
         DS_CHECK(flush_alpha());
-        FOR_SLABS(s) DS_CHECK(launch_rhs(s.g, lc, s.q, s.alpha, s.c, s.weight, s.u0_prev, s.w0, s.st));
+        FOR_SLABS(s) DS_CHECK(launch_rhs(s.g, lc, s.q, s.alpha, s.c, s.weight, s.u0_prev, s.w0, s.st, c_ends_on && s.c_ends));
     } else if (multi()) {
         FOR_SLABS(s)
             if (!s.g.first) DS_CHECK(launch_rhs_fixup(s.g, lc, s.u0_prev, s.w0, s.st));
@@ -1275,7 +1311,13 @@
         prof_end(PH_PROJ);
         return 0;
     }
-    const int ph = deferred ? PH_FUSED_B : PH_FUSED_A;
+    const bool gin = beta_gamma, gout = deferred && cone_gout;
+    if (gin && (!deferred || bpend)) {
+        set_error("internal: gamma form %s", deferred ? "with a pending scaling of beta" : "without a pending multiplier step");
+        return DOTSOCP_ESTATE;
+    }
+    const int flavour = (gin ? CONE_GIN : 0) | (gout ? CONE_GOUT : 0);
+    const int ph = deferred ? (gin ? PH_CONE_CARRY : PH_FUSED_B) : PH_FUSED_A;
     z_valid = false;
     z_prev_ok = false;
     prof_begin(ph);
@@ -1299,16 +1341,19 @@
             for (i64 z = z0; z < z0 + zc; ++z) {
                 a.carry_in = (z > 0) ? s.carry : nullptr;
                 a.carry_out = (z + 1 < C) ? s.carry : nullptr;
-                DS_CHECK(launch_cone_fused(mode, s.g, lc, s.fg, a, s.st, z, 1));
+                DS_CHECK(launch_cone_fused(mode, s.g, lc, s.fg, a, s.st, z, 1, flavour));
             }
         } else {
-            DS_CHECK(launch_cone_fused(mode, s.g, lc, s.fg, a, s.st, z0, zc));
+            DS_CHECK(launch_cone_fused(mode, s.g, lc, s.fg, a, s.st, z0, zc, flavour));
         }
         if (deferred && part != 1) std::swap(s.beta, s.beta2);
     }
     prof_end(ph);
     if (part == 1) return 0;
-    if (deferred) bpend = 0;
+    if (deferred) {
+        bpend = 0;
+        beta_gamma = gout;
+    }
     return 0;
 }
 
@@ -1377,6 +1422,7 @@
                 else if (part == 2) { z0 = C - 1; zc = 1; }
                 QStepExtra ex{};
                 ex.apend = apend ? 1 : 0; ex.amul = amul; ex.adiv = adiv;
+                ex.c_ends = (c_ends_on && s.c_ends) ? 1 : 0;
                 if (multi() && !s.g.last && part != 1) ex.u0_tail = s.send_plane;
                 if (kkt) {
                     const KktCoef k = kkt_coef();
@@ -1417,6 +1463,7 @@
 
 int Solver::materialise() {
     if (!fused || !deferred) return 0;
+    DS_CHECK(need_beta_form("materialise"));
     DS_CHECK(ensure_halo());
     prof_begin(PH_MATERIALISE);
     FOR_SLABS(s) {
@@ -1438,6 +1485,7 @@
 
 int Solver::ensure_z() {
     if (!fused || z_valid) return 0;
+    DS_CHECK(need_beta_form("ensure_z"));
     if (deferred) return materialise();
     if (!z_prev_ok) {
         set_error("internal: z cannot be regenerated");
@@ -1461,6 +1509,7 @@
 }
 
 int Solver::kkt_sums(double *S, bool folded) {
+    DS_CHECK(need_beta_form("kkt_sums"));
     DS_CHECK(ensure_halo());
     const KktCoef k = kkt_coef();
     if (method == DOTSOCP_METHOD_ACCADMM && folded) {
@@ -1553,6 +1602,7 @@
 }
 
 int Solver::norms_light(double *S) {
+    DS_CHECK(need_beta_form("norms_light"));
     DS_CHECK(ensure_halo());
     DS_CHECK(flush_alpha());
     const KktCoef k = kkt_coef();
@@ -1591,6 +1641,7 @@
         nAlps = std::max(normAlpha, normBeta);
         return 0;
     };
+    if (rescale_due(it, rescale, maxFeas, relGap)) DS_CHECK(need_beta_form("rescale_block"));
     if (rescale >= 3 && (it % 100) == 0) {
         DS_CHECK(norms(normPhis, normAlps));
         const double ratio = std::max(normAlps, normPhis) / std::min(normAlps, normPhis);
@@ -1615,6 +1666,20 @@
     update_coef();
     rescale += 1;
     return 0;
+}
+
+bool rescale_due(i64 it, int rescale, double maxFeas, double relGap) {
+    if (rescale >= 3 && (it % 100) == 0) return true;
+    if (rescale == 1 && maxFeas < 2e-2 && it >= 10 && relGap < 5e-2) return true;
+    if (rescale == 2 && maxFeas < 5e-3 && it >= 50 && relGap < 1e-2) return true;
+    return false;
+}
+
+bool cone_writes_beta(i64 it, double lastSigmaIt, i64 maxit, bool checkStepByStep, bool last_of_run, int rescale,
+                      double maxFeas, double relGap) {
+    if (checkStepByStep || if_adjust_sigma((double)it, lastSigmaIt) || it >= maxit) return true;
+    if (last_of_run) return true;
+    return rescale_due(it + 1, rescale, maxFeas, relGap);
 }
 
 bool if_adjust_sigma(double iter, double last_iter) {
@@ -1727,7 +1792,9 @@
     it += 1;
     DS_CHECK(rescale_block());
     const bool adjustSigmaYes = if_adjust_sigma((double)it, lastSigmaIt);
-    const bool kkt_due = opts.ifCheckStepByStep || adjustSigmaYes || it == opts.maxit;
+    const bool kkt_due = opts.ifCheckStepByStep || adjustSigmaYes || it == opts.maxit || timeout_pending;
+    cone_gout = cone_carry && fused && deferred && !kkt_due &&
+                !cone_writes_beta(it, lastSigmaIt, opts.maxit, opts.ifCheckStepByStep != 0, last_of_run, rescale, maxFeas, relGap);
     const bool fold = kkt_due && kkt_fold && fused && qrhs;
     const bool inter = comm_z && multi() && fused && qrhs;
     bool split = inter && cone_split_enabled();
@@ -1776,7 +1843,12 @@
         DS_CHECK(phase_q(0, fold));
     }
     DS_CHECK(phase_mult());
-    const bool timed_out = remote() ? false : (elapsed() > time_limit);
+    const bool timed_out = timeout_pending || (remote() ? false : (elapsed() > time_limit || (timeout_at > 0 && it >= timeout_at)));
+    timeout_pending = false;
+    if (timed_out && beta_gamma) {
+        timeout_pending = true;
+        return 0;
+    }
     if (kkt_due || timed_out)
         DS_CHECK(kkt_block(adjustSigmaYes, timed_out, brk, fold));
     return 0;
@@ -1797,10 +1869,12 @@
     while (it < opts.maxit && !stopped) {
         if (n_iters >= 0 && n >= n_iters) break;
         bool brk = false;
+        last_of_run = (n_iters >= 0 && n + 1 >= n_iters);
         DS_CHECK(step(&brk));
         if (brk) stopped = true;
         ++n;
     }
+    DS_CHECK(need_beta_form("the end of run()"));
     DS_CHECK(ensure_halo());
     DS_CHECK(sync_all());
     DS_CHECK(prof_flush());
@@ -1838,7 +1912,7 @@
         res->cScale = cScale;
         res->dScale = dScale;
         res->times[0] = (phase_ms[PH_RHS] + phase_ms[PH_POISSON]) * 1e-3;
-        res->times[1] = (phase_ms[PH_PROJ] + phase_ms[PH_FUSED_A] + phase_ms[PH_FUSED_B]) * 1e-3;
+        res->times[1] = (phase_ms[PH_PROJ] + phase_ms[PH_FUSED_A] + phase_ms[PH_FUSED_B] + phase_ms[PH_CONE_CARRY]) * 1e-3;
         res->times[2] = phase_ms[PH_QSTEP] * 1e-3;
         res->times[3] = (phase_ms[PH_BETA] + phase_ms[PH_MATERIALISE]) * 1e-3;
         res->times[4] = phase_ms[PH_KKT] * 1e-3;
diff --git a/dot-socp_amd/csrc/solver_io.hip b/dot-socp_amd/csrc/solver_io.hip
--- a/dot-socp_amd/csrc/solver_io.hip
+++ b/dot-socp_amd/csrc/solver_io.hip
@@ -8,6 +8,7 @@
 int Solver::recover_outputs(const double *rho0, const double *rho1, double *rho, double *Ex, double *Ey, double *q0,
                             double *bx, double *by) {
     if (!finished) { set_error("recover_outputs() needs finish()"); return DOTSOCP_ESTATE; }
+    DS_CHECK(need_beta_form("recover_outputs"));
     DS_ARG(rho == nullptr || (rho0 != nullptr && rho1 != nullptr), "rho needs rho0 and rho1");
     cur_dev = -1;
     DS_CHECK(use_dev(device));
diff --git a/dot-socp_amd/csrc/stencil.hip b/dot-socp_amd/csrc/stencil.hip
--- a/dot-socp_amd/csrc/stencil.hip
+++ b/dot-socp_amd/csrc/stencil.hip
@@ -19,9 +19,9 @@
 }
 
 int launch_rhs(const Grid &g, const LoopCoef &c, const double *q, const double *alpha, const double *cvec,
-               const double *weight, const double *u0_prev, double *rhs, hipStream_t st) {
+               const double *weight, const double *u0_prev, double *rhs, hipStream_t st, bool c_ends) {
     if (g.Nphi <= 0) return 0;
-    RhsArgs a{g, c.at, c.ax, c.ay, q, alpha, cvec, weight, u0_prev};
+    RhsArgs a{g, c.at, c.ax, c.ay, q, alpha, cvec, weight, u0_prev, c_ends ? 1 : 0};
     if (weight)
         DS_KLAUNCH(k_rhs<true>, tile_grid(g, g.ntl), dim3(TILE_Y, TILE_X), 0, st, a, rhs);
     else
@@ -343,6 +343,7 @@
     const double *qk;
     double *partials, *resid;
     double kappa, dsD;
+    int c_ends;
 };
 
 enum { Q_Q2 = 0, Q_ALPHA2, Q_APHI2, Q_PRIM1, Q_QALPHA, Q_CPHI, Q_PHI2, Q_DUAL1, Q_MRHOB, Q_M2, Q_RHOB2, Q_COUNT };
@@ -455,7 +456,8 @@
         double k0v = 0.0, kXv = 0.0, kYv = 0.0;
         const bool pcorr = (VAR == 3) && (a.qk != nullptr);
         if (pcorr) { k0v = a.qk[k0]; kXv = a.qk[eX]; kYv = a.qk[eY]; }
-        const double cv = a.cvec[node];
+        double cv = 0.0;
+        if (!a.c_ends || tbnd) cv = a.cvec[node];
         double w0 = 1.0, wX = 1.0, wY = 1.0;
         if (WEIGHTED) { w0 = a.weight[k0]; wX = a.weight[eX]; wY = a.weight[eY]; }
         const double sxv = a.sx[sxOwn ? (tl * fg.nxblk + (x / fg.XB + 1)) * g.ny + y : 0];
@@ -689,6 +691,7 @@
         a.u0_tail = ex->u0_tail;
         a.kappa = ex->kappa;
         a.dsD = ex->dsD;
+        a.c_ends = ex->c_ends;
     }
     return launch_qstep_rhs_var(0, g, c, fg, a, st, z0, zcount, zstride);
 }
@@ -696,17 +699,43 @@
 i64 qstep_rhs_blocks(const Grid &g, const FusedGeom &fg) { return fg.nyblk * fg.nxblk * qstep_rhs_chunks(g, fg); }
 
 __global__ void __launch_bounds__(256) k_rhs_sigma_fix(double *__restrict__ rhs, const double *__restrict__ r,
-                                                        double *__restrict__ cvec, i64 n, double factor) {
+                                                        double *__restrict__ cvec, i64 n, double factor, i64 c_lo, i64 c_hi) {
     for (i64 i = (i64)blockIdx.x * blockDim.x + threadIdx.x; i < n; i += (i64)gridDim.x * blockDim.x) {
         const double rv = r[i];
         rhs[i] = (rhs[i] + rv) - rv / factor;
-        cvec[i] = cvec[i] / factor;
-    }
-}
-
-int launch_rhs_sigma_fix(double *rhs, const double *r, double *cvec, i64 n, double factor, hipStream_t st) {
+        if (i < c_lo || i >= c_hi) cvec[i] = cvec[i] / factor;
+    }
+}
+
+static inline void c_interior(const Grid &g, i64 &c_lo, i64 &c_hi) {
+    c_lo = g.first ? g.plane : 0;
+    c_hi = g.last ? g.Nphi - g.plane : g.Nphi;
+    if (c_hi < c_lo) c_hi = c_lo;
+}
+
+int launch_rhs_sigma_fix(const Grid &g, double *rhs, const double *r, double *cvec, double factor, hipStream_t st,
+                         bool c_ends) {
+    const i64 n = g.Nphi;
     if (n <= 0) return 0;
-    DS_KLAUNCH(k_rhs_sigma_fix, dim3(launch_blocks(n, 256, 1 << 22)), dim3(256), 0, st, rhs, r, cvec, n, factor);
+    i64 c_lo = n, c_hi = n;
+    if (c_ends) c_interior(g, c_lo, c_hi);
+    DS_KLAUNCH(k_rhs_sigma_fix, dim3(launch_blocks(n, 256, 1 << 22)), dim3(256), 0, st, rhs, r, cvec, n, factor, c_lo, c_hi);
+    DS_HIP(hipGetLastError());
+    return 0;
+}
+
+__global__ void __launch_bounds__(256) k_any_nonzero_bits(const double *__restrict__ c, i64 lo, i64 hi, int *flag) {
+    bool any = false;
+    for (i64 i = lo + (i64)blockIdx.x * blockDim.x + threadIdx.x; i < hi; i += (i64)gridDim.x * blockDim.x)
+        any = any || (__double_as_longlong(c[i]) != 0);
+    if (any) atomicOr(flag, 1);
+}
+
+int launch_c_interior_test(const Grid &g, const double *cvec, int *flag, hipStream_t st) {
+    i64 lo, hi;
+    c_interior(g, lo, hi);
+    if (hi <= lo) return 0;
+    DS_KLAUNCH(k_any_nonzero_bits, dim3(launch_blocks(hi - lo, 256, 1 << 14)), dim3(256), 0, st, cvec, lo, hi, flag);
     DS_HIP(hipGetLastError());
     return 0;
 }
diff --git a/include/dotsocp.h b/include/dotsocp.h
--- a/include/dotsocp.h
+++ b/include/dotsocp.h
@@ -114,6 +114,10 @@
 
 int dotsocp_dct_algorithm(dotsocp_i64 n);
 
+int dotsocp_cone_writes_beta(dotsocp_i64 it, double last_sigma_it, dotsocp_i64 maxit, int check_step_by_step,
+                             int last_of_run, int rescale, double maxFeas, double relGap);
+int dotsocp_rescale_due(dotsocp_i64 it, int rescale, double maxFeas, double relGap);
+
 int dotsocp_upload(dotsocp_ctx *ctx, int field, const double *host);
 int dotsocp_download(dotsocp_ctx *ctx, int field, double *host);
 int dotsocp_upload_layers(dotsocp_ctx *ctx, int field, const double *host, dotsocp_i64 t0, dotsocp_i64 n);
```

After: 85.63 (median of 6 runs). 5.3% higher.
